# izhengfan/se2lam

Hardware: AMD Instinct MI355X
Metric: BA GN-iters/s (200 KF, 20k pts) (higher is better)
Workload: dtype f64; 1 GPU; globalBA-window 200 KF / 20000 landmarks / 119817 EdgeSE2XYZ + 199 PreEdgeSE2, LM optimize(10) (config 4 formulation, SURVEY D3); parallelism=single GPU

## Files before the change

include/se2gpu.h:

```cpp
#ifndef SE2GPU_H
#define SE2GPU_H

#include <stddef.h>
#include <stdint.h>

#ifdef __cplusplus
extern "C" {
#endif

#define SE2GPU_OK 0
#define SE2GPU_ERR_INVALID (-1)
#define SE2GPU_ERR_NO_DEVICE (-2)
#define SE2GPU_ERR_HIP (-3)
#define SE2GPU_ERR_CAPACITY (-4)
#define SE2GPU_ERR_STATE (-5)

const char* se2gpu_last_error(void);
int se2gpu_device_count(void);
const char* se2gpu_version(void);

typedef struct se2gpu_orb se2gpu_orb;

typedef struct se2gpu_orb_params {
    int32_t nfeatures;
// ... 88 lines not shown
int se2gpu_ba_clear(se2gpu_ba* h);
int se2gpu_ba_set_stream(se2gpu_ba* h, void* hip_stream);
int se2gpu_ba_add_cam(se2gpu_ba* h, double f, double cx, double cy);
int se2gpu_ba_set_Tbc(se2gpu_ba* h, const double R[9], const double t[3]);
int se2gpu_ba_add_vertex_se2(se2gpu_ba* h, int id, double x, double y, double theta, int fixed);
int se2gpu_ba_add_vertex_xyz(se2gpu_ba* h, int id, const double xyz[3], int marginal, int fixed);
int se2gpu_ba_add_edge_se2xyz(se2gpu_ba* h, int id_kf, int id_mp, const double uv[2], const double info[4],
                              double huber_delta);
int se2gpu_ba_add_edge_se2(se2gpu_ba* h, int id0, int id1, const double meas[3], const double info[9]);

int se2gpu_ba_load(se2gpu_ba* h, int P, int L, int E, int O,
                   const double* poses, const uint8_t* fixed, const double* lms,
                   const int32_t* e_kf, const int32_t* e_lm, const double* e_uv, const double* e_info,
                   const int32_t* o_i, const int32_t* o_j, const double* o_meas, const double* o_info,
                   double huber_delta);

int se2gpu_ba_add_vertex_se3(se2gpu_ba* h, int id, const double pose12[12], int fixed);
int se2gpu_ba_add_vertex_iso3(se2gpu_ba* h, int id, const double Twc12[12], int fixed);
int se2gpu_plane_motion_prior_iso3(const double* Twc12, const double* Tbc12, double xrot_info, double yrot_info,
                                   double z_info, double* meas12, double* info36);
int se2gpu_ba_add_prior_se3(se2gpu_ba* h, int id, const double meas12[12], const double info36[36]);
int se2gpu_ba_add_edge_se3(se2gpu_ba* h, int id0, int id1, const double meas12[12], const double info36[36]);
int se2gpu_ba_add_edge_xyz2uv(se2gpu_ba* h, int id_mp, int id_kf, const double uv[2], double inv_sigma2, double huber_delta);
int se2gpu_ba_get_se3(se2gpu_ba* h, int id, double pose12[12]);
int se2gpu_ba_edge_chi2(se2gpu_ba* h, double* chi2, int cap);

int se2gpu_sparsify_se3xyz(int npairs, const double* kf12, const int32_t* mp_ptr, const double* mp_xyz,
                           const int32_t* m_ptr, const int32_t* m_kf, const int32_t* m_mp, const double* m_info,
                           double* z_out12, double* info_out36);

typedef struct se2gpu_local_graph {
    int32_t n_local_kf, n_ref_kf, n_mp, n_obs;
    const int32_t* kf_id;
    const float* kf_Twb;
    const float* kf_Rcw;
    const int32_t* odo_to;
    const double* odo_meas;
    const double* odo_cov;
    const float* mp_pos;
    const int32_t* obs_mp;
    const int32_t* obs_kf;
    const float* obs_uv;
    const float* obs_lc;
    const float* obs_sigma2;
    float fx, cx, cy;
    double Rbc[9], tbc[3];
    float huber_delta;
    float xrot_info, z_info;
} se2gpu_local_graph;
int se2gpu_ba_load_local_graph(se2gpu_ba* h, const se2gpu_local_graph* graph);

typedef struct se2gpu_map_view {
    int32_t n_kf, n_mp;
    const int32_t* kf_id;
    const int32_t* covis_ptr; const int32_t* covis_idx;
    const int32_t* kf_mp_ptr; const int32_t* kf_mp_idx;
    const int32_t* mp_id;
    const int32_t* mp_kf_ptr; const int32_t* mp_kf_idx;
} se2gpu_map_view;
int se2gpu_map_update_local_graph(const se2gpu_map_view* map, int current_kf, int search_level, int32_t* local_kfs,
                                  int* n_local, int32_t* ref_kfs, int* n_ref, int32_t* local_mps, int* n_mps);

int se2gpu_ba_initialize(se2gpu_ba* h);
int se2gpu_ba_set_edge_level(se2gpu_ba* h, int edge, int level);
int se2gpu_ba_reset_estimates(se2gpu_ba* h);
int se2gpu_ba_reset_estimates_batch(se2gpu_ba** handles, int count);

#define SE2GPU_BA_LM 0
#define SE2GPU_BA_GN 1
int se2gpu_ba_optimize(se2gpu_ba* h, int iters, int mode, const volatile uint8_t* stop_flag, int verbose,
                       se2gpu_ba_stats* stats);
int se2gpu_ba_optimize_batch(se2gpu_ba** handles, int count, int iters, int mode, const volatile uint8_t* stop_flag,
                             se2gpu_ba_stats* stats);
int se2gpu_ba_last_batch_path(void);
int se2gpu_ba_get_se2(se2gpu_ba* h, int id, double xyt[3]);
int se2gpu_ba_get_xyz(se2gpu_ba* h, int id, double xyz[3]);
int se2gpu_ba_get_all(se2gpu_ba* h, double* poses , double* lms );
double se2gpu_ba_chi2(se2gpu_ba* h);

int se2gpu_ba_debug_reduced_system(se2gpu_ba* h, double lambda, double* S, double* bs);
int se2gpu_ba_debug_solve(se2gpu_ba* h, double lambda, double* x, int* factor_ok);
int se2gpu_ba_debug_solver_path(const se2gpu_ba* h);
int se2gpu_ba_debug_linearize_counts(const se2gpu_ba* h, int* runs, int* skips, long long* twin_bytes);
int se2gpu_ba_debug_pool_sizes(int out2[2]);
int se2gpu_ba_debug_chol_verify(se2gpu_ba* h, unsigned long long* counts2, unsigned long long* records, int cap);
int se2gpu_ba_debug_solve_plan(int P, int D, const uint8_t* pattern, int allow_nd, int* nsys, int* nbc, int* depth, int* ntask,
                               int* ndep, int32_t* pose_off, int32_t* tasks4, int task_cap, int32_t* deps, int dep_cap);
int se2gpu_ba_debug_solve_plan_tile(int P, int D, const uint8_t* pattern, int allow_nd, int tile, int* nsys, int* nbc, int* depth, int* ntask,
                                    int* ndep, int32_t* pose_off, int32_t* tasks4, int task_cap, int32_t* deps, int dep_cap);

int se2gpu_triangulate(int n, const se2gpu_keypoint* kps_ref, const se2gpu_keypoint* kps_cur, int n_cur,
                       int32_t* match_idx, const uint8_t* has_observation, const float* P_ref, const float* P_cur,
                       const float* Ocam, float lower_depth, float upper_depth, int min_degree, float* pos_out,
                       uint8_t* good_parallax, int* n_good, int* n_tracked_old);

typedef struct se2gpu_track se2gpu_track;
int se2gpu_track_create(se2gpu_track** out);
void se2gpu_track_destroy(se2gpu_track* h);
int se2gpu_track_fundamental_mask(se2gpu_track* h, const float* pt1, const float* pt2, int n, uint8_t* mask,
                                  int* n_inliers);
int se2gpu_track_remove_outliers(se2gpu_track* h, const se2gpu_keypoint* kps1, int n1, const se2gpu_keypoint* kps2,
                                 int n2, int32_t* matches, int* n_inliers);
int se2gpu_track_last_ransac(const se2gpu_track* h, int info[4]);
int se2gpu_track_triangulate(se2gpu_track* h, int n, const se2gpu_keypoint* kps_ref, const se2gpu_keypoint* kps_cur,
                             int n_cur, int32_t* match_idx, const uint8_t* has_observation, const float* P_ref,
                             const float* P_cur, const float* Ocam, float lower_depth, float upper_depth,
                             int min_degree, float* pos_out, uint8_t* good_parallax, int* n_good, int* n_tracked_old);

int se2gpu_plane_motion_prior(const double* Tcw12, const double* Tbc12, double xrot_info, double yrot_info, double z_info,
                              double* meas12, double* info36);
int se2gpu_track_pose_ba(se2gpu_track* h, const double* Tcw12, const double* prior_meas12, const double* prior_info36, int n,
                         const double* xyz, const double* uv, const double* inv_sigma2, double f, double cx, double cy,
                         double huber_delta, int iters, double* Tcw_out12, se2gpu_ba_stats* stats);

int se2gpu_ba_edge_information(int E, const float* lc, const float* lw, const int32_t* e_kf, const float* sigma2, int P,
                               const float* Rcw, const float* twb_xy, float fx, float xrot_info, float z_info,
                               double* info_out);

typedef int (*se2gpu_allreduce_fn)(void* dev_ptr, size_t count_doubles, void* hip_stream, void* user);
size_t se2gpu_ba_reduce_buffer_doubles(se2gpu_ba* h, int P);
size_t se2gpu_ba_exchange_doubles(int P);
size_t se2gpu_ba_exchange_doubles_h(const se2gpu_ba* h);
int se2gpu_ba_exchange_row(int row, size_t* offset, int* length);
int se2gpu_ba_set_allreduce(se2gpu_ba* h, se2gpu_allreduce_fn fn, void* user, void* buffer);
int se2gpu_ba_set_shard(se2gpu_ba* h, int rank, int world);

typedef struct se2gpu_comm se2gpu_comm;
int se2gpu_comm_unique_id(uint8_t id_out[128]);
int se2gpu_comm_create(const uint8_t id[128], int rank, int world, se2gpu_comm** out);
int se2gpu_comm_count(se2gpu_comm* c, int* nranks);
void se2gpu_comm_destroy(se2gpu_comm* c);
int se2gpu_comm_allreduce_sum_f64(se2gpu_comm* c, void* dev_ptr, size_t count, void* hip_stream);
int se2gpu_ba_set_comm(se2gpu_ba* h, se2gpu_comm* c);

int se2gpu_ba_shard_landmarks(int L, int E, const int32_t* e_kf, const int32_t* e_lm, int world, int32_t* owner);

typedef struct se2gpu_timer se2gpu_timer;
int se2gpu_timer_create(se2gpu_timer** out);
void se2gpu_timer_destroy(se2gpu_timer* t);
int se2gpu_timer_start(se2gpu_timer* t, void* hip_stream);
int se2gpu_timer_stop(se2gpu_timer* t, void* hip_stream);
int se2gpu_timer_elapsed_ms(se2gpu_timer* t, float* ms);
void* se2gpu_orb_stream(se2gpu_orb* h);
void* se2gpu_matcher_stream(se2gpu_matcher* h);
void* se2gpu_ba_stream(se2gpu_ba* h);
int se2gpu_ba_profile(se2gpu_ba* h, int enable);
int se2gpu_ba_profile_get(se2gpu_ba* h, int idx, const char** name, double* ms, int64_t* launches);
int se2gpu_orb_score_kernel(se2gpu_orb* h, int info[2]);
int se2gpu_orb_profile(se2gpu_orb* h, int enable);
int se2gpu_orb_profile_get(se2gpu_orb* h, int idx, const char** name, double* ms, int64_t* launches);

int se2gpu_malloc(void** dev_ptr, size_t bytes);
int se2gpu_free(void* dev_ptr);
int se2gpu_memcpy_h2d(void* dst, const void* src, size_t bytes);
int se2gpu_memcpy_d2h(void* dst, const void* src, size_t bytes);
int se2gpu_device_synchronize(void);
int se2gpu_set_device(int ordinal);
int se2gpu_host_alloc(void** host_ptr, size_t bytes);
int se2gpu_host_free(void* host_ptr);
int se2gpu_memcpy_h2d_async(void* dst, const void* src, size_t bytes, void* hip_stream);
int se2gpu_memcpy_d2h_async(void* dst, const void* src, size_t bytes, void* hip_stream);
int se2gpu_stream_create(void** hip_stream_out);
int se2gpu_stream_destroy(void* hip_stream);
int se2gpu_stream_synchronize(void* hip_stream);
int se2gpu_timer_stream_wait(se2gpu_timer* t, void* hip_stream);

// ... 5 lines not shown
```

se2lam_amd/capi.py:

```python
from __future__ import annotations

import ctypes as C
import os

import numpy as np

HERE = os.path.dirname(os.path.abspath(__file__))
LIB_PATH = os.path.join(HERE, "lib", "libse2gpu.so")

OK = 0
ERR_INVALID, ERR_NO_DEVICE, ERR_HIP, ERR_CAPACITY, ERR_STATE = -1, -2, -3, -4, -5


class Se2GpuError(RuntimeError):
    def __init__(self, code, msg):
        super().__init__(f"se2gpu error {code}: {msg}")
        self.code = code


class Keypoint(C.Structure):
    _fields_ = [("x", C.c_float), ("y", C.c_float), ("size", C.c_float), ("angle", C.c_float),
                ("response", C.c_float), ("octave", C.c_int32), ("class_id", C.c_int32)]


# ... 35 lines not shown
                ("lambda_final", C.c_double), ("chi2_hist", C.c_double * 64), ("lambda_hist", C.c_double * 64),
                ("trials_hist", C.c_int32 * 64)]


ALLREDUCE_FN = C.CFUNCTYPE(C.c_int, C.c_void_p, C.c_size_t, C.c_void_p, C.c_void_p)

_VP, _I, _D, _F, _SZ = C.c_void_p, C.c_int, C.c_double, C.c_float, C.c_size_t
_PD, _PI32, _PU8, _PF = C.POINTER(C.c_double), C.POINTER(C.c_int32), C.POINTER(C.c_uint8), C.POINTER(C.c_float)
_PKP = C.POINTER(Keypoint)
SYMBOLS = {
    "se2gpu_last_error": (C.c_char_p, []),
    "se2gpu_device_count": (_I, []),
    "se2gpu_version": (C.c_char_p, []),
    "se2gpu_orb_create": (_I, [C.POINTER(OrbParams), C.POINTER(_VP)]),
    "se2gpu_orb_destroy": (None, [_VP]),
    "se2gpu_orb_levels": (_I, [_VP]),
    "se2gpu_orb_scale_factor": (_F, [_VP]),
    "se2gpu_orb_extract": (_I, [_VP, _VP, _I, _I, _SZ, _VP, _VP, _VP, _I, C.POINTER(_I)]),
    "se2gpu_orb_extract_batch_device": (_I, [_VP, _VP, _I, _I, _I, _VP, _VP, _VP, _I]),
    "se2gpu_orb_sync": (_I, [_VP]),
    "se2gpu_orb_set_stream": (_I, [_VP, _VP]),
    "se2gpu_orb_debug_level": (_I, [_VP, _I, _I, _I, _VP, _SZ, C.POINTER(_I), C.POINTER(_I)]),
    "se2gpu_orb_debug_score": (_I, [_VP, _I, _I, _VP, _SZ, C.POINTER(_I), C.POINTER(_I)]),
    "se2gpu_orb_debug_nth_element": (_I, [_VP, _I, _I, _I]),
    "se2gpu_orb_stream": (_VP, [_VP]),
    "se2gpu_orb_score_kernel": (_I, [_VP, _VP]),
    "se2gpu_orb_profile": (_I, [_VP, _I]),
    "se2gpu_orb_profile_get": (_I, [_VP, _I, C.POINTER(C.c_char_p), _PD, C.POINTER(C.c_int64)]),
    "se2gpu_hamming": (_I, [_VP, _VP]),
    "se2gpu_three_maxima": (_I, [_VP, _I, _VP, _VP, _VP]),
    "se2gpu_matcher_create": (_I, [_I, _I, C.POINTER(_VP)]),
    "se2gpu_matcher_destroy": (None, [_VP]),
    "se2gpu_matcher_set_stream": (_I, [_VP, _VP]),
    "se2gpu_matcher_sync": (_I, [_VP]),
    "se2gpu_matcher_spill_calls": (_I, [_VP, _VP]),
    "se2gpu_matcher_stream": (_VP, [_VP]),
    "se2gpu_match_window": (_I, [_VP, C.POINTER(FrameBounds), _VP, _VP, _I, _VP, _VP, _I, _VP, _I, _I, _I, _I, _F,
                                 _VP, C.POINTER(_I)]),
    "se2gpu_match_window_batch_device": (_I, [_VP, C.POINTER(FrameBounds), _VP, _VP, _VP, _I, _VP, _VP, _I, _I, _I,
                                              _I, _I, _F, _VP, _VP]),
    "se2gpu_search_by_bow": (_I, [_VP, _VP, _VP, _I, _VP, _VP, _VP, _I, _VP, _VP, _VP, _I, _VP, _VP, _VP, _I, _VP, _I, _F, _I,
                                  _VP, C.POINTER(_I)]),
    "se2gpu_match_projection": (_I, [_VP, C.POINTER(FrameBounds), _VP, _VP, _VP, _VP, _I, _VP, _F, _F, _F, _F,
                                     _VP, _VP, _VP, _I, _I, _I, _F, _VP, C.POINTER(_I)]),
    "se2gpu_ba_create": (_I, [C.POINTER(_VP)]),
    "se2gpu_ba_reserve": (_I, [_I, _I, _I]),
    "se2gpu_ba_destroy": (None, [_VP]),
    "se2gpu_ba_clear": (_I, [_VP]),
    "se2gpu_ba_set_stream": (_I, [_VP, _VP]),
    "se2gpu_ba_stream": (_VP, [_VP]),
    "se2gpu_ba_add_cam": (_I, [_VP, _D, _D, _D]),
    "se2gpu_ba_set_Tbc": (_I, [_VP, _PD, _PD]),
    "se2gpu_ba_add_vertex_se2": (_I, [_VP, _I, _D, _D, _D, _I]),
    "se2gpu_ba_add_vertex_xyz": (_I, [_VP, _I, _PD, _I, _I]),
    "se2gpu_ba_add_edge_se2xyz": (_I, [_VP, _I, _I, _PD, _PD, _D]),
    "se2gpu_ba_add_edge_se2": (_I, [_VP, _I, _I, _PD, _PD]),
    "se2gpu_ba_load": (_I, [_VP, _I, _I, _I, _I, _PD, _PU8, _PD, _PI32, _PI32, _PD, _PD, _PI32, _PI32, _PD, _PD, _D]),
    "se2gpu_ba_load_local_graph": (_I, [_VP, C.POINTER(LocalGraph)]),
    "se2gpu_ba_add_vertex_se3": (_I, [_VP, _I, _PD, _I]),
    "se2gpu_ba_add_vertex_iso3": (_I, [_VP, _I, _PD, _I]),
    "se2gpu_plane_motion_prior_iso3": (_I, [_VP, _VP, _D, _D, _D, _VP, _VP]),
    "se2gpu_ba_add_prior_se3": (_I, [_VP, _I, _PD, _PD]),
    "se2gpu_ba_add_edge_se3": (_I, [_VP, _I, _I, _PD, _PD]),
    "se2gpu_ba_add_edge_xyz2uv": (_I, [_VP, _I, _I, _PD, _D, _D]),
    "se2gpu_ba_get_se3": (_I, [_VP, _I, _PD]),
    "se2gpu_ba_edge_chi2": (_I, [_VP, _PD, _I]),
    "se2gpu_map_update_local_graph": (_I, [C.POINTER(MapView), _I, _I, _VP, C.POINTER(_I), _VP, C.POINTER(_I), _VP, C.POINTER(_I)]),
    "se2gpu_sparsify_se3xyz": (_I, [_I, _VP, _VP, _VP, _VP, _VP, _VP, _VP, _VP, _VP]),
    "se2gpu_ba_initialize": (_I, [_VP]),
    "se2gpu_ba_set_edge_level": (_I, [_VP, _I, _I]),
    "se2gpu_ba_reset_estimates": (_I, [_VP]),
    "se2gpu_ba_reset_estimates_batch": (_I, [_VP, _I]),
    "se2gpu_ba_optimize": (_I, [_VP, _I, _I, _PU8, _I, C.POINTER(BaStats)]),
    "se2gpu_ba_optimize_batch": (_I, [C.POINTER(_VP), _I, _I, _I, _PU8, C.POINTER(BaStats)]),
    "se2gpu_ba_last_batch_path": (_I, []),
    "se2gpu_ba_get_se2": (_I, [_VP, _I, _PD]),
    "se2gpu_ba_get_xyz": (_I, [_VP, _I, _PD]),
    "se2gpu_ba_get_all": (_I, [_VP, _PD, _PD]),
    "se2gpu_ba_chi2": (_D, [_VP]),
    "se2gpu_ba_debug_reduced_system": (_I, [_VP, _D, _PD, _PD]),
    "se2gpu_ba_debug_solve": (_I, [_VP, _D, _PD, C.POINTER(C.c_int)]),
    "se2gpu_ba_debug_solver_path": (_I, [_VP]),
    "se2gpu_ba_debug_linearize_counts": (_I, [_VP, C.POINTER(C.c_int), C.POINTER(C.c_int), C.POINTER(C.c_longlong)]),
    "se2gpu_ba_debug_chol_verify": (_I, [_VP, _VP, _VP, _I]),
    "se2gpu_ba_debug_pool_sizes": (_I, [_VP]),
    "se2gpu_ba_debug_solve_plan": (_I, [_I, _I, _VP, _I, _VP, _VP, _VP, _VP, _VP, _VP, _VP, _I, _VP, _I]),
    "se2gpu_ba_debug_solve_plan_tile": (_I, [_I, _I, _VP, _I, _I, _VP, _VP, _VP, _VP, _VP, _VP, _VP, _I, _VP, _I]),
    "se2gpu_triangulate": (_I, [_I, _VP, _VP, _I, _VP, _VP, _VP, _VP, _VP, C.c_float, C.c_float, _I, _VP, _VP,
                           C.POINTER(C.c_int), C.POINTER(C.c_int)]),
    "se2gpu_track_create": (_I, [C.POINTER(_VP)]),
    "se2gpu_track_destroy": (None, [_VP]),
    "se2gpu_track_fundamental_mask": (_I, [_VP, _VP, _VP, _I, _VP, C.POINTER(C.c_int)]),
    "se2gpu_track_remove_outliers": (_I, [_VP, _VP, _I, _VP, _I, _VP, C.POINTER(C.c_int)]),
    "se2gpu_track_last_ransac": (_I, [_VP, _VP]),
    "se2gpu_plane_motion_prior": (_I, [_VP, _VP, _D, _D, _D, _VP, _VP]),
    "se2gpu_track_pose_ba": (_I, [_VP, _VP, _VP, _VP, _I, _VP, _VP, _VP, _D, _D, _D, _D, _I, _VP, C.POINTER(BaStats)]),
    "se2gpu_track_triangulate": (_I, [_VP, _I, _VP, _VP, _I, _VP, _VP, _VP, _VP, _VP, C.c_float, C.c_float, _I, _VP, _VP,
                                 C.POINTER(C.c_int), C.POINTER(C.c_int)]),
    "se2gpu_ba_reduce_buffer_doubles": (_SZ, [_VP, _I]),
    "se2gpu_ba_exchange_doubles": (_SZ, [_I]),
    "se2gpu_ba_exchange_doubles_h": (_SZ, [_VP]),
    "se2gpu_ba_exchange_row": (_I, [_I, C.POINTER(C.c_size_t), C.POINTER(C.c_int)]),
    "se2gpu_ba_set_allreduce": (_I, [_VP, ALLREDUCE_FN, _VP, _VP]),
    "se2gpu_ba_set_shard": (_I, [_VP, _I, _I]),
    "se2gpu_comm_unique_id": (_I, [_VP]),
    "se2gpu_comm_create": (_I, [_VP, _I, _I, C.POINTER(_VP)]),
    "se2gpu_comm_destroy": (None, [_VP]),
    "se2gpu_comm_count": (_I, [_VP, C.POINTER(_I)]),
    "se2gpu_comm_allreduce_sum_f64": (_I, [_VP, _VP, _SZ, _VP]),
    "se2gpu_ba_set_comm": (_I, [_VP, _VP]),
    "se2gpu_ba_shard_landmarks": (_I, [_I, _I, _PI32, _PI32, _I, _PI32]),
    "se2gpu_ba_edge_information": (_I, [_I, _VP, _VP, _VP, _VP, _I, _VP, _VP, _F, _F, _F, _VP]),
    "se2gpu_ba_profile": (_I, [_VP, _I]),
    "se2gpu_ba_profile_get": (_I, [_VP, _I, C.POINTER(C.c_char_p), _PD, C.POINTER(C.c_int64)]),
    "se2gpu_timer_create": (_I, [C.POINTER(_VP)]),
    "se2gpu_timer_destroy": (None, [_VP]),
    "se2gpu_timer_start": (_I, [_VP, _VP]),
    "se2gpu_timer_stop": (_I, [_VP, _VP]),
    "se2gpu_timer_elapsed_ms": (_I, [_VP, C.POINTER(C.c_float)]),
    "se2gpu_malloc": (_I, [C.POINTER(_VP), _SZ]),
    "se2gpu_free": (_I, [_VP]),
    "se2gpu_memcpy_h2d": (_I, [_VP, _VP, _SZ]),
    "se2gpu_memcpy_d2h": (_I, [_VP, _VP, _SZ]),
    "se2gpu_host_alloc": (_I, [C.POINTER(_VP), _SZ]),
    "se2gpu_host_free": (_I, [_VP]),
    "se2gpu_memcpy_h2d_async": (_I, [_VP, _VP, _SZ, _VP]),
    "se2gpu_memcpy_d2h_async": (_I, [_VP, _VP, _SZ, _VP]),
    "se2gpu_stream_create": (_I, [C.POINTER(_VP)]),
    "se2gpu_stream_destroy": (_I, [_VP]),
    "se2gpu_stream_synchronize": (_I, [_VP]),
    "se2gpu_timer_stream_wait": (_I, [_VP, _VP]),
    "se2gpu_device_synchronize": (_I, []),
    "se2gpu_set_device": (_I, [_I]),
}

_lib = None


def lib() -> C.CDLL:
    global _lib
    if _lib is None:
        if not os.path.exists(LIB_PATH):
            raise ImportError(
                f"{LIB_PATH} is missing - run `python -m se2lam_amd.build` (or __graft_entry__.build()). "
                "se2lam_amd has no CPU / eager fallback.")
        l = C.CDLL(LIB_PATH)
        for name, (res, args) in SYMBOLS.items():
            fn = getattr(l, name)
            fn.restype = res
            fn.argtypes = args
        _lib = l
    return _lib


def check(rc: int):
    if rc != OK:
        raise Se2GpuError(rc, lib().se2gpu_last_error().decode(errors="replace"))


def device_count() -> int:
    return int(lib().se2gpu_device_count())


def vp(a: np.ndarray) -> C.c_void_p:
    return C.c_void_p(a.ctypes.data)

# ... 100 lines not shown
```

se2lam_amd/csrc/ba.hip:

```cpp
#include <algorithm>
#include <atomic>
#include <chrono>
#include <cmath>
#include <cstdlib>
#include <functional>
#include <limits>
#include <mutex>
#include <thread>
#include <tuple>
#include <memory>
#include <unordered_map>

#include "common.h"
#include "se3_math.h"
#include "ba_device.h"
#include "ba3_device.h"
#include "ba_window.h"

using namespace se2gpu;
using namespace se2gpu::badev;

namespace {


// ... 839 lines not shown
        __syncthreads();
    } else {
        t0 = *reinterpret_cast<const double2*>(ownp);
        t1 = *reinterpret_cast<const double2*>(ownp + 2);
        const double* dp = A + (size_t)r * ld + cc;
        d0 = *reinterpret_cast<const double2*>(dp);
        d1 = *reinterpret_cast<const double2*>(dp + 2);
        if (!elim) return;
    }
    Ti[r][cc] = t0.x; Ti[r][cc + 1] = t0.y; Ti[r][cc + 2] = t1.x; Ti[r][cc + 3] = t1.y;
    Tj[r][cc] = d0.x; Tj[r][cc + 1] = d0.y; Tj[r][cc + 2] = d1.x; Tj[r][cc + 3] = d1.y;
    __syncthreads();
    if (tid >= 64) return;
    const int lane = tid;
    const int c0 = kNB * k;
    const int ncol = min(kNB, n - c0);
    const int rr = lane & 31;
    double m[kNB];
    {
        const double* lp = (lane < kNB) ? &Tj[rr][0] : &Ti[rr][0];
        const bool ident = isDiag && lane >= kNB;
#pragma unroll
        for (int c = 0; c < kNB; c += 2) {
            const double2 v = *reinterpret_cast<const double2*>(lp + c);
            m[c] = ident ? (c == rr ? 1.0 : 0.0) : v.x;
            m[c + 1] = ident ? (c + 1 == rr ? 1.0 : 0.0) : v.y;
        }
#pragma unroll
        for (int c = 0; c < kNB; ++c)
            if (c >= ncol) m[c] = (lane < kNB && c == rr) ? 1e300 : 0.0;
    }
    double inv = fast_rcp(bcast_lane(m[0], 0));
#pragma unroll
    for (int jj = 0; jj < kNB; ++jj) {
        const double mr = m[jj] * inv;
        if (jj + 1 < kNB) {
            m[jj + 1] = fma(-mr, bcast_lane(m[jj], jj + 1), m[jj + 1]);
            inv = fast_rcp(bcast_lane(m[jj + 1], jj + 1));
        }
        if (jj + 2 < kNB) {
            double* col = (jj & 1) ? colB : colA;
            col[lane] = m[jj];
#pragma unroll
            for (int c = jj + 2; c < kNB; ++c) m[c] = fma(-mr, col[c], m[c]);
        }
    }
    bool bad = false;
    double out[kNB];
#pragma unroll
    for (int c = 0; c < kNB; ++c) {
        const double d = bcast_lane(m[c], c);
        const bool pos = (d > 0.0) & (d < __builtin_inf());
        bad |= (c < ncol) & !pos;
        out[c] = m[c] * fast_rsqrt(((c < ncol) & pos) ? d : 1.0);
    }
    double* rowp;
    if (lane < kNB) rowp = A + (size_t)(c0 + rr) * ld + c0;
    else if (isDiag) rowp = R + (size_t)(c0 + rr) * ld + c0;
    else rowp = own + (size_t)(kNB * i + rr) * ld + c0;
    if (ncol == kNB) {
        if (lane >= kNB) {
            double2* wp2 = reinterpret_cast<double2*>(rowp);
#pragma unroll
            for (int c = 0; c < kNB; c += 2) wp2[c / 2] = make_double2(out[c], out[c + 1]);
        }
    } else {
#pragma unroll
        for (int c = 0; c < kNB; ++c)
            if (c < ncol && (lane >= kNB || (isDiag && rr >= ncol))) rowp[c] = out[c];
    }
    if (bad && isDiag && lane == 0) fail[0] = 1.0;
}

typedef double d2_t __attribute__((ext_vector_type(2)));
typedef double d4_t __attribute__((ext_vector_type(4)));
__device__ inline d2_t load_agent(const double* p) {
    d2_t v;
    asm volatile("global_load_dwordx4 %0, %1, off sc1" : "=v"(v) : "v"(p) : "memory");
    return v;
}
__device__ inline void store_agent(double* p, d2_t v) {
    asm volatile("global_store_dwordx4 %0, %1, off sc1\n\ts_nop 1" : : "v"(p), "v"(v) : "memory");
}
#define SE2_WAIT_VM6(a, b, c, d, e, f) \
    asm volatile("s_waitcnt vmcnt(0)" : "+v"(a), "+v"(b), "+v"(c), "+v"(d), "+v"(e), "+v"(f) : : "memory")

__device__ inline unsigned poll_agent(const unsigned* p) {
    unsigned v;
    asm volatile("global_load_dword %0, %1, off sc1" : "=v"(v) : "v"(p) : "memory");
    return v;
}
__device__ inline bool spin_until(const unsigned* f, unsigned epoch, bool lazy = false) {
    if (__hip_atomic_load(f, __ATOMIC_RELAXED, __HIP_MEMORY_SCOPE_AGENT) == epoch) return true;
    const long long t0 = wall_clock64();
    while (__hip_atomic_load(f, __ATOMIC_RELAXED, __HIP_MEMORY_SCOPE_AGENT) != epoch) {
        if (lazy) __builtin_amdgcn_s_sleep(48);
        else __builtin_amdgcn_s_sleep(2);
        if (wall_clock64() - t0 > 200000000ll) return false;
    }
    return true;
}

constexpr int kVfyRecords = 64, kVfyChk = 8 + 8 * kVfyRecords;
__device__ inline unsigned long long wave_xor64(unsigned long long v) {
#pragma unroll
    for (int m = 1; m < 64; m <<= 1) v ^= (unsigned long long)__shfl_xor((long long)v, m);
    return v;
}
__device__ inline unsigned long long bits4(d2_t a, d2_t b) {
    return (unsigned long long)__double_as_longlong(a.x) ^ (unsigned long long)__double_as_longlong(a.y) ^
           (unsigned long long)__double_as_longlong(b.x) ^ (unsigned long long)__double_as_longlong(b.y);
}
template <bool VERIFY>
__device__ __forceinline__ void d_chol_tiles(const unsigned bx_dispatch, const double* __restrict__ A, double* __restrict__ PUB,
                                                     double* __restrict__ YU, int ld, int n,
                                                     int nbc, const int4* __restrict__ tasks, const int* __restrict__ deps,
                                                     const int* __restrict__ col_src,
                                                     unsigned* __restrict__ flagA, unsigned* __restrict__ flagR,
                                                     const unsigned* __restrict__ epoch_ptr, double* __restrict__ fail,
                                                     long long* __restrict__ dbg, const BaCtl* __restrict__ ctl,
                                                     double* __restrict__ xout, unsigned long long* __restrict__ vfy,
                                                     unsigned long long* __restrict__ head, int ntask) {
    if (ctl && ctl->done) return;
    __shared__ unsigned task_s;
    if (head) {
        if (threadIdx.x == 0) {
            const unsigned c = __hip_atomic_fetch_add(reinterpret_cast<unsigned*>(head), 1u, __ATOMIC_RELAXED, __HIP_MEMORY_SCOPE_AGENT);
            if (c == (unsigned)ntask - 1u) __hip_atomic_store(reinterpret_cast<unsigned*>(head), 0u, __ATOMIC_RELAXED, __HIP_MEMORY_SCOPE_AGENT);
            task_s = c;
        }
        __syncthreads();
    }
    const unsigned bx = head ? task_s : bx_dispatch;
    const unsigned epoch = *epoch_ptr;
    const int nt = ld / kNB;
    constexpr int kTile = kNB * (kNB + 2);
    __shared__ __attribute__((aligned(16))) double LD[3 * kTile + kNB * kNB + 8 * kNB];
    double (*Tb)[kNB + 2] = reinterpret_cast<double (*)[kNB + 2]>(LD);
    double (*Tc)[kNB + 2] = reinterpret_cast<double (*)[kNB + 2]>(LD + kTile);
    double (*Ta)[kNB + 2] = reinterpret_cast<double (*)[kNB + 2]>(LD + 2 * kTile);
    double (*COLV)[kNB] = reinterpret_cast<double (*)[kNB]>(LD + 3 * kTile);
    double* const DUMMY = LD + 3 * kTile + kNB * kNB;
    double (*MRC)[64] = reinterpret_cast<double (*)[64]>(LD + kTile);
    static_assert(16 * 64 <= kTile && 32 * 64 <= 2 * kTile, "rows 0..15 of MRC lie inside Tc, all of it inside Tc | Ta");
    __shared__ int ok_s, ready_s, loaded_s, slab_s[kSlabs];
    __shared__ int deps_s[64];
    const int tid = threadIdx.x;
    if (tid == 0) { ready_s = 0; loaded_s = 0; ok_s = 1; }
    if (tid < kSlabs) slab_s[tid] = 0;
    long long* stamp = dbg ? dbg + (size_t)bx * 16 : nullptr;
    if (stamp && tid == 0) stamp[0] = wall_clock64();
    const int4 tk = tasks[bx];
    if (tid < tk.w - tk.z && tid < 64) deps_s[tid] = deps[tk.z + tid];
    __syncthreads();
    if ((tk.x >> 16) == 2) {
        const int r = tk.x & 0xffff;
        const int it = n / kNB;
        const int row = tid / 8, c4 = (tid % 8) * 4;
        double acc = 0.0;
        for (int dq = tk.z; dq < tk.w; ++dq) {
            const int j = deps_s[dq - tk.z];
            if (tid == 0) {
                const bool lazy = dq + 1 < tk.w;
                bool ok = true;
                for (int sl = 0; sl < kSlabs; ++sl) {
                    ok = ok && spin_until(flagR + ((size_t)r * nbc + j) * kSlabs + sl, epoch, lazy);
// ... 227 lines not shown
    if (stamp && tid == 224) stamp[6] = clock64() - clk0;
    if (lane >= kNB) {
        double* pb = PUB + pub_tile(isR || isDiag ? 1 : 0, i, j, nt, nbc) + w * kSlabDoubles + rr * 2;
#pragma unroll
        for (int q = 0; q < 8; q += 2) {
            store_agent(pb + q * kNB, d2_t{m[q], m[q + 1]});
            store_agent(pb + kSlabDoubles / 2 + q * kNB, d2_t{mrs[q], mrs[q + 1]});
        }
    }
    if constexpr (VERIFY) {
        unsigned long long xm = 0, xr = 0;
        if (lane >= kNB) {
#pragma unroll
            for (int q = 0; q < 8; ++q) {
                xm ^= (unsigned long long)__double_as_longlong(m[q]);
                xr ^= (unsigned long long)__double_as_longlong(mrs[q]);
            }
        }
        xm = wave_xor64(xm);
        xr = wave_xor64(xr);
        if (lane == 0) {
            const size_t tx = ((size_t)((isR || isDiag ? 1 : 0) * nt + i) * nbc + j) * kSlabs + w;
            __hip_atomic_store(vfy + kVfyChk + 2 * tx, xm, __ATOMIC_RELAXED, __HIP_MEMORY_SCOPE_AGENT);
            __hip_atomic_store(vfy + kVfyChk + 2 * tx + 1, xr, __ATOMIC_RELAXED, __HIP_MEMORY_SCOPE_AGENT);
        }
    }
    if (!isR && i == n / kNB && lane == (isDiag ? 0 : kNB) + n % kNB) {
#pragma unroll
        for (int q = 0; q < 8; q += 2) store_agent(YU + c0 + cb + q, d2_t{m[q], m[q + 1]});
    }
    if (bad && isDiag && lane == 0) fail[0] = 1.0;
    asm volatile("s_waitcnt vmcnt(0)" ::: "memory");
    if (lane == 0)
        __hip_atomic_store((isR || isDiag ? flagR : flagA) + ((size_t)i * nbc + j) * kSlabs + w, epoch, __ATOMIC_RELAXED, __HIP_MEMORY_SCOPE_AGENT);
    if (stamp && lane == 0) stamp[12 + w] = wall_clock64();
    if (stamp && tid == 192) stamp[5] = wall_clock64();
}
template <bool VERIFY>
__global__ __launch_bounds__(256) void k_chol_tiles(const double* __restrict__ A, double* __restrict__ PUB,
                                                     double* __restrict__ YU, int ld, int n,
                                                     int nbc, const int4* __restrict__ tasks, const int* __restrict__ deps,
                                                     const int* __restrict__ col_src,
                                                     unsigned* __restrict__ flagA, unsigned* __restrict__ flagR,
                                                     const unsigned* __restrict__ epoch_ptr, double* __restrict__ fail,
                                                     long long* __restrict__ dbg, const BaCtl* __restrict__ ctl,
                                                     double* __restrict__ xout, unsigned long long* __restrict__ vfy,
                                                     unsigned long long* __restrict__ head, int ntask) {
    d_chol_tiles<VERIFY>(blockIdx.x, A, PUB, YU, ld, n, nbc, tasks, deps, col_src, flagA, flagR, epoch_ptr, fail, dbg, ctl, xout, vfy, head, ntask);
}

__global__ __launch_bounds__(256) void k_chol_apply(const double* __restrict__ A, const double* __restrict__ R, int ld,
                                                     int n, double* __restrict__ x, const BaCtl* __restrict__ ctl,
                                                     const int* __restrict__ col_src) {
    if (ctl && ctl->done) return;
    const int r = blockIdx.x * 4 + threadIdx.x / 64;
    const int lane = threadIdx.x & 63;
    if (r >= n) return;
    const double* y = A + (size_t)n * ld;
    double acc = 0.0;
    for (int c = r + lane; c < n; c += 64) acc += R[(size_t)r * ld + c] * y[c];
    acc = wave_sum(acc);
    const int dst = col_src ? col_src[r] : r;
    if (lane == 0 && dst >= 0) x[dst] = acc;
}

struct FinArgs {
    int enabled, nblk, P, O, root, step, decide, notify;
    const uint8_t* fixed;
    const double* xp;
    const double* bp;
    const double* poses;
    double* poses_trial;
    const int* o_i;
    const int* o_j;
    const double* o_meas;
    const double* o_info;
    double* out;
    volatile double* mail;
    double seq;
    BaCtl* ctl;
    const volatile int* stop;
    unsigned* counter;
    int spec;
};
__device__ void finish_trial(const FinArgs& fin, const double* part, double lambda, double* fsp);

struct SpecArgs {
    RecSet set[2];
    double *Hpp_e, *bp_e;
};

template <bool LIN>
__device__ __forceinline__ void d_update(const unsigned bx, CamDev cam, int L, double lambda, const int* __restrict__ lm_ptr,
                                                    const int* __restrict__ e_kf, const double* __restrict__ e_uv,
                                                    const double* __restrict__ e_info,
                                                    const double* __restrict__ poses,
                                                    const uint8_t* __restrict__ fixed, const double* __restrict__ lms,
                                                    const double* __restrict__ xp, const double* __restrict__ zeta,
                                                    const double* __restrict__ W, const double* __restrict__ bl,
                                                    double* __restrict__ lms_trial, double* __restrict__ part,
                                                    const BaCtl* __restrict__ ctl, const double* __restrict__ poses_b,
                                                    FinArgs fin, const double* __restrict__ Ainv, SpecArgs sp) {
    __shared__ double lds[LIN ? (kBlock / 64) * kWaveLds : 3 * 1024];
    static_assert((kBlock / 64) * kWaveLds >= 3 * 1024, "the finisher's pose stage");
    if (fin.enabled && (int)bx == fin.nblk) {
        finish_trial(fin, part, lambda, lds);
        return;
    }
    const int gid = bx * kBlock + threadIdx.x;
    const int l = gid / kGroup, sub = gid % kGroup;
    int beg = 0, end = 0;
    if (l < L) {
        beg = lm_ptr[l];
        end = lm_ptr[l + 1];
    }
    if (ctl) {
        if (ctl->done) return;
        if (ctl->sel) {
            const double* t = lms; lms = lms_trial; lms_trial = const_cast<double*>(t);
            poses = poses_b;
        }
        lambda = ctl->lambda;
    }
    const bool step = xp != nullptr;
    bool spec = false;
    double lambda_spec = 0;
    RecSet wr{};
    if (LIN && ctl && step) {
        spec = ctl->it + 1 < ctl->iters;
        lambda_spec = lm_lambda_spec(lambda, ctl->mode);
        const int rs = ctl->rec_sel;
        const RecSet rd = sp.set[rs];
        wr = sp.set[rs ^ 1];
        W = rd.W; zeta = rd.zeta; bl = rd.bl; Ainv = rd.Ainv;
    }
    double* keep = lds;
    double hll[6] = {0, 0, 0, 0, 0, 0}, bsum[3] = {0, 0, 0};
    __shared__ double sm[2][kBlock / 64];
    double chi = 0, scale = 0;
    double x[3] = {0, 0, 0};
    constexpr int KS = 2;
    int ekf[KS];
    bool ev[KS];
    double ey[KS][9], ep[KS][3], epose[KS][3], euv[KS][2], ew[KS][3];
    bool efix[KS];
#pragma unroll
    for (int k = 0; k < KS; ++k) {
        const int e = beg + sub + k * kGroup;
        ev[k] = e < end;
        const int ec = ev[k] ? e : max(end - 1, 0);
        const bool has = l < L && end > beg;
        ekf[k] = has ? e_kf[ec] : 0;
#pragma unroll
        for (int i = 0; i < 9; ++i) ey[k][i] = (has && step) ? W[(size_t)ec * 9 + i] : 0.0;
        euv[k][0] = has ? e_uv[2 * (size_t)ec] : 0.0;
        euv[k][1] = has ? e_uv[2 * (size_t)ec + 1] : 0.0;
#pragma unroll
        for (int i = 0; i < 3; ++i) ew[k][i] = has ? e_info[3 * (size_t)ec + i] : 0.0;
    }
#pragma unroll
    for (int k = 0; k < KS; ++k) {
        const int kf = ekf[k];
        epose[k][0] = poses[3 * kf]; epose[k][1] = poses[3 * kf + 1]; epose[k][2] = poses[3 * kf + 2];
        efix[k] = fixed[kf] != 0;
#pragma unroll
        for (int i = 0; i < 3; ++i) ep[k][i] = step ? xp[3 * kf + i] : 0.0;
    }
    double lw0[3] = {0, 0, 0}, zz[3] = {0, 0, 0}, blv[3] = {0, 0, 0}, av[6] = {0, 0, 0, 0, 0, 0};
    if (l < L) {
#pragma unroll
        for (int c = 0; c < 3; ++c) {
            lw0[c] = lms[(size_t)l * 3 + c];
            if (step) { zz[c] = zeta[(size_t)l * 3 + c]; blv[c] = bl[(size_t)l * 3 + c]; }
        }
        if (step) {
#pragma unroll
            for (int c = 0; c < 6; ++c) av[c] = Ainv[(size_t)l * 6 + c];
        }
    }
    if (l < L && step) {
#pragma unroll
        for (int k = 0; k < KS; ++k)
            if (ev[k]) {
#pragma unroll
                for (int c = 0; c < 3; ++c) x[c] -= ey[k][c] * ep[k][0] + ey[k][3 + c] * ep[k][1] + ey[k][6 + c] * ep[k][2];
            }
        for (int e = beg + sub + KS * kGroup; e < end; e += kGroup) {
            const int kf = e_kf[e];
            const double* y = W + (size_t)e * 9;
            const double p0 = xp[3 * kf], p1 = xp[3 * kf + 1], p2 = xp[3 * kf + 2];
#pragma unroll
            for (int c = 0; c < 3; ++c) x[c] -= y[c] * p0 + y[3 + c] * p1 + y[6 + c] * p2;
        }
    }
#pragma unroll
    for (int c = 0; c < 3; ++c) x[c] = group_sum(x[c]);
    if (l < L && step) {
        const double t0 = zz[0] + x[0], t1 = zz[1] + x[1], t2 = zz[2] + x[2];
        x[0] = av[0] * t0 + av[1] * t1 + av[3] * t2;
        x[1] = av[2] * t1 + av[4] * t2;
        x[2] = av[5] * t2;
    }
    if (l < L) {
        double lw[3];
#pragma unroll
        for (int c = 0; c < 3; ++c) lw[c] = lw0[c] + x[c];
        if (sub == 0 && step) {
#pragma unroll
            for (int c = 0; c < 3; ++c) {
                lms_trial[(size_t)l * 3 + c] = lw[c];
                scale += x[c] * (lambda * x[c] + blv[c]);
            }
        }
        auto edge_chi = [&](int e, double px, double py, double pth, bool fx, const double* dp, double u, double v, double w0,
                            double w1, double w2) {
            if (step && !fx) {
                px += dp[0];
                py += dp[1];
                pth = normalize_theta(pth + dp[2]);
            }
            if (LIN && spec) {
                double hpl[9], hpp[6], bpe[3], r0;
                lin_edge(cam, px, py, pth, lw[0], lw[1], lw[2], u, v, w0, w1, w2, !fx, hll, bsum, hpl, hpp, bpe, r0);
                chi += r0;
                lin_park<true>(e == beg + sub, e, hpl, hpp, bpe, keep, wr.W, sp.Hpp_e, sp.bp_e);
                return;
            }
            double e0, e1;
            se2xyz<false>(cam, px, py, pth, lw[0], lw[1], lw[2], u, v, e0, e1, nullptr, nullptr);
            double r0, r1;
            huber(e0 * (w0 * e0 + w1 * e1) + e1 * (w1 * e0 + w2 * e1), cam.huber, r0, r1);
            chi += r0;
        };
#pragma unroll
        for (int k = 0; k < KS; ++k)
            if (ev[k]) edge_chi(beg + sub + k * kGroup, epose[k][0], epose[k][1], epose[k][2], efix[k], ep[k], euv[k][0], euv[k][1], ew[k][0], ew[k][1], ew[k][2]);
        for (int e = beg + sub + KS * kGroup; e < end; e += kGroup) {
            const int kf = e_kf[e];
            double dp[3] = {0, 0, 0};
            if (step) { dp[0] = xp[3 * kf]; dp[1] = xp[3 * kf + 1]; dp[2] = xp[3 * kf + 2]; }
            edge_chi(e, poses[3 * kf], poses[3 * kf + 1], poses[3 * kf + 2], fixed[kf] != 0, dp, e_uv[2 * e], e_uv[2 * e + 1],
                     e_info[3 * e], e_info[3 * e + 1], e_info[3 * e + 2]);
        }
    }
    chi = wave_sum(chi);
    scale = wave_sum(scale);
    const int w = threadIdx.x / 64;
    if ((threadIdx.x & 63) == 0) { sm[0][w] = chi; sm[1][w] = scale; }
    __syncthreads();
    if (threadIdx.x == 0) {
        double c = 0, s = 0;
        for (int i = 0; i < kBlock / 64; ++i) { c += sm[0][i]; s += sm[1][i]; }
        if (fin.enabled) {
            store_agent(part + 2 * bx, d2_t{c, s});
            asm volatile("s_waitcnt vmcnt(0)" ::: "memory");
            __hip_atomic_fetch_add(fin.counter, 1u, __ATOMIC_RELAXED, __HIP_MEMORY_SCOPE_AGENT);
        } else {
            part[2 * bx] = c;
            part[2 * bx + 1] = s;
        }
    }
    if (LIN && spec)
        lin_landmark<true>(l, sub, beg, end, L, hll, bsum, lambda_spec, keep, wr.W, sp.Hpp_e, sp.bp_e, wr.Hll, wr.bl, wr.Ainv,
                           wr.zeta, wr.Dg);
}
template <bool LIN>
__global__ __launch_bounds__(kBlock) void k_update(CamDev cam, int L, double lambda, const int* __restrict__ lm_ptr,
                                                    const int* __restrict__ e_kf, const double* __restrict__ e_uv,
                                                    const double* __restrict__ e_info,
                                                    const double* __restrict__ poses,
                                                    const uint8_t* __restrict__ fixed, const double* __restrict__ lms,
                                                    const double* __restrict__ xp, const double* __restrict__ zeta,
                                                    const double* __restrict__ W, const double* __restrict__ bl,
                                                    double* __restrict__ lms_trial, double* __restrict__ part,
                                                    const BaCtl* __restrict__ ctl, const double* __restrict__ poses_b,
                                                    FinArgs fin, const double* __restrict__ Ainv, SpecArgs sp) {
    d_update<LIN>(blockIdx.x, cam, L, lambda, lm_ptr, e_kf, e_uv, e_info, poses, fixed, lms, xp, zeta, W, bl, lms_trial, part, ctl, poses_b, fin, Ainv, sp);
}


__global__ void k_ctl_clear_error(BaCtl* __restrict__ ctl) {
    ctl->error = 0;
    ctl->done = 0;
}

__device__ inline void post_ctl(const BaCtl* c, volatile double* mail, double seq, int tid, int nthr) {
    constexpr int kWords = (int)(sizeof(BaCtl) / 8);
    const double* src = reinterpret_cast<const double*>(c);
    for (int i = tid; i < kWords; i += nthr) mail[8 + i] = src[i];
}

__device__ inline void end_slot(BaCtl* ctl, volatile double* mail, bool post, int tid, int nthr, bool step) {
    if (!step) return;
    if (tid == 0) ctl->seq += 1.0;
    __syncthreads();
    if (post && mail) {
        __threadfence();
        post_ctl(ctl, mail, 0.0, tid, nthr);
        __threadfence_system();
        __syncthreads();
        if (tid == 0) mail[kMailSeq] = ctl->seq;
    }
}

__device__ void finish_trial(const FinArgs& fin, const double* part, double lambda, double* fsp) {
    __shared__ double fsm[2][kBlock / 64];
    __shared__ int fpost;
    BaCtl* ctl = fin.ctl;
    const volatile double* cmail = fin.mail;
    volatile double* mail = fin.mail;
    (void)cmail;
    const double* poses = fin.poses;
    double* poses_trial = fin.poses_trial;
    const bool step = fin.step != 0;
    int stopped = 0;
    double failflag = 0;
    if (ctl) {
        if (ctl->done) {
            end_slot(ctl, mail, fin.notify != 0, threadIdx.x, blockDim.x, fin.step != 0);
            return;
        }
        if (ctl->sel) { const double* t = poses; poses = poses_trial; poses_trial = const_cast<double*>(t); }
        lambda = ctl->lambda;
    }
    if (threadIdx.x == 0) {
        stopped = (fin.stop && *fin.stop) ? 1 : 0;
        failflag = step ? fin.out[2] : 0.0;
    }
    double chi = 0, scale = 0;
    for (int p = threadIdx.x; p < fin.P; p += blockDim.x) {
        double x = poses[3 * p], y = poses[3 * p + 1], th = poses[3 * p + 2];
        if (step && !fin.fixed[p]) {
            const double d0 = fin.xp[3 * p], d1 = fin.xp[3 * p + 1], d2 = fin.xp[3 * p + 2];
            x += d0; y += d1; th = normalize_theta(th + d2);
            const double* bp = fin.bp;
            if (fin.root) scale += d0 * (lambda * d0 + bp[3 * p]) + d1 * (lambda * d1 + bp[3 * p + 1]) + d2 * (lambda * d2 + bp[3 * p + 2]);
            else scale += d0 * bp[3 * p] + d1 * bp[3 * p + 1] + d2 * bp[3 * p + 2];
        }
        if (step) { poses_trial[3 * p] = x; poses_trial[3 * p + 1] = y; poses_trial[3 * p + 2] = th; }
        if (p < 1024) { fsp[3 * p] = x; fsp[3 * p + 1] = y; fsp[3 * p + 2] = th; }
    }
    __syncthreads();
    for (int k = threadIdx.x; k < fin.O; k += blockDim.x) {
        const int i = fin.o_i[k], j = fin.o_j[k];
        double pi[3], pj[3];
        for (int c = 0; c < 3; ++c) {
            pi[c] = (i < 1024) ? fsp[3 * i + c] : (step ? poses_trial[3 * i + c] : poses[3 * i + c]);
            pj[c] = (j < 1024) ? fsp[3 * j + c] : (step ? poses_trial[3 * j + c] : poses[3 * j + c]);
        }
        double e[3], A[9], B[9];
        pre_se2(pi, pj, fin.o_meas + 3 * k, e, A, B);
        const double* W = fin.o_info + 9 * k;
        for (int r = 0; r < 3; ++r) chi += e[r] * (W[r * 3] * e[0] + W[r * 3 + 1] * e[1] + W[r * 3 + 2] * e[2]);
    }
    if (threadIdx.x == 0) {
        const long long t0 = wall_clock64();
        while (__hip_atomic_load(fin.counter, __ATOMIC_RELAXED, __HIP_MEMORY_SCOPE_AGENT) != (unsigned)fin.nblk) {
            __builtin_amdgcn_s_sleep(1);
            if (wall_clock64() - t0 > 200000000ll) break;
        }
        __hip_atomic_store(fin.counter, 0u, __ATOMIC_RELAXED, __HIP_MEMORY_SCOPE_AGENT);
    }
    __syncthreads();
    for (int i0 = threadIdx.x; i0 < fin.nblk; i0 += 4 * blockDim.x) {
        d2_t v[4];
#pragma unroll
        for (int u = 0; u < 4; ++u) v[u] = load_agent(part + 2 * min(i0 + u * (int)blockDim.x, fin.nblk - 1));
        asm volatile("s_waitcnt vmcnt(0)" : "+v"(v[0]), "+v"(v[1]), "+v"(v[2]), "+v"(v[3]) : : "memory");
#pragma unroll
        for (int u = 0; u < 4; ++u)
            if (i0 + u * (int)blockDim.x < fin.nblk) { chi += v[u].x; scale += v[u].y; }
    }
    chi = wave_sum(chi);
    scale = wave_sum(scale);
    if ((threadIdx.x & 63) == 0) {
        fsm[0][threadIdx.x >> 6] = chi;
        fsm[1][threadIdx.x >> 6] = scale;
    }
    __syncthreads();
    if (threadIdx.x == 0) {
        for (int w = 1; w < (int)(blockDim.x >> 6); ++w) {
            fsm[0][0] += fsm[0][w];
            fsm[1][0] += fsm[1][w];
        }
        double* out = fin.out;
        out[0] = fsm[0][0]; out[1] = fsm[1][0]; out[3] = 0;
        if (!step) out[2] = 0;
        fpost = 0;
        if (ctl && fin.decide) {
            if (!step) {
                ctl->current_chi = ctl->chi2_init = ctl->chi2_final = fsm[0][0];
                if (stopped) { ctl->stopped = 1; ctl->done = 1; }
                if (ctl->iters <= 0) ctl->done = 1;
            } else {
                const double sc[3] = {fsm[0][0], fsm[1][0], failflag};
                const int sel0 = ctl->sel;
                const bool speculated = fin.spec && ctl->it + 1 < ctl->iters;
                const double lambda_spec = lm_lambda_spec(ctl->lambda, ctl->mode);
                lm_advance(ctl, sc, stopped != 0);
                if (!ctl->error) lm_records_advance(ctl, speculated, sel0, lambda_spec);
            }
            fpost = (ctl->done || fin.notify) && mail;
        } else if (mail && !ctl) {
            mail[0] = fsm[0][0];
            mail[1] = fsm[1][0];
            mail[2] = step ? failflag : 0.0;
            __threadfence_system();
            mail[3] = fin.seq;
        }
    }
    if (ctl && fin.decide) {
        __syncthreads();
        end_slot(ctl, mail, fpost != 0, threadIdx.x, blockDim.x, step);
    }
}

__global__ void k_finalize(int nparts, const double* __restrict__ part, int P, double lambda,
                           const double* __restrict__ poses, const uint8_t* __restrict__ fixed,
                           const double* __restrict__ xp, const double* __restrict__ bp, double* __restrict__ poses_trial,
                           int O, const int* __restrict__ o_i, const int* __restrict__ o_j,
                           const double* __restrict__ o_meas, const double* __restrict__ o_info, int root,
                           double* __restrict__ out, volatile double* __restrict__ mail, double seq,
                           BaCtl* __restrict__ ctl, int step_arg, int decide, int notify,
                           const volatile int* __restrict__ stop) {
    __shared__ double sm[2][16];
    __shared__ double sp[3 * 1024];
    __shared__ int post_s;
    bool step = xp != nullptr;
    if (ctl) {
        step = step_arg != 0;
        if (ctl->done) {
            if (decide) end_slot(ctl, mail, notify != 0, threadIdx.x, blockDim.x, step);
            return;
        }
        if (ctl->sel) { const double* t = poses; poses = poses_trial; poses_trial = const_cast<double*>(t); }
        lambda = ctl->lambda;
    }
    double chi = 0, scale = 0;
    for (int i = threadIdx.x; i < nparts; i += blockDim.x) {
        chi += part[2 * i];
        scale += part[2 * i + 1];
    }
    for (int p = threadIdx.x; p < P; p += blockDim.x) {
        double x = poses[3 * p], y = poses[3 * p + 1], th = poses[3 * p + 2];
        if (step && !fixed[p]) {
            const double d0 = xp[3 * p], d1 = xp[3 * p + 1], d2 = xp[3 * p + 2];
            x += d0; y += d1; th = normalize_theta(th + d2);
            if (root) scale += d0 * (lambda * d0 + bp[3 * p]) + d1 * (lambda * d1 + bp[3 * p + 1]) + d2 * (lambda * d2 + bp[3 * p + 2]);
            else scale += d0 * bp[3 * p] + d1 * bp[3 * p + 1] + d2 * bp[3 * p + 2];
        }
        if (step) { poses_trial[3 * p] = x; poses_trial[3 * p + 1] = y; poses_trial[3 * p + 2] = th; }
        if (p < 1024) { sp[3 * p] = x; sp[3 * p + 1] = y; sp[3 * p + 2] = th; }
    }
    __syncthreads();
    for (int k = threadIdx.x; k < O; k += blockDim.x) {
        const int i = o_i[k], j = o_j[k];
        double pi[3], pj[3];
        for (int c = 0; c < 3; ++c) {
            pi[c] = (i < 1024) ? sp[3 * i + c] : (step ? poses_trial[3 * i + c] : poses[3 * i + c]);
            pj[c] = (j < 1024) ? sp[3 * j + c] : (step ? poses_trial[3 * j + c] : poses[3 * j + c]);
        }
        double e[3], A[9], B[9];
        pre_se2(pi, pj, o_meas + 3 * k, e, A, B);
        const double* W = o_info + 9 * k;
        for (int r = 0; r < 3; ++r) chi += e[r] * (W[r * 3] * e[0] + W[r * 3 + 1] * e[1] + W[r * 3 + 2] * e[2]);
    }
    chi = wave_sum(chi);
    scale = wave_sum(scale);
    if ((threadIdx.x & 63) == 0) {
        sm[0][threadIdx.x >> 6] = chi;
        sm[1][threadIdx.x >> 6] = scale;
    }
    __syncthreads();
    if (threadIdx.x == 0) {
        for (int w = 1; w < (int)(blockDim.x >> 6); ++w) {
            sm[0][0] += sm[0][w];
            sm[1][0] += sm[1][w];
        }
        out[0] = sm[0][0]; out[1] = sm[1][0]; out[3] = 0;
        if (!step) out[2] = 0;
        post_s = 0;
        if (ctl && decide) {
            if (!step) {
// ... 868 lines not shown
    int find(int id) const {
        if ((unsigned)id < dense.size()) return dense[(unsigned)id];
        if ((unsigned)id < kDenseIds) return -1;
        const auto it = sparse.find(id);
        return it == sparse.end() ? -1 : it->second;
    }
    void set(int id, int slot) {
        if ((unsigned)id < kDenseIds) {
            if ((unsigned)id >= dense.size()) dense.resize(std::max<size_t>((size_t)id + 1, 2 * dense.size()), -1);
            dense[(unsigned)id] = slot;
        } else {
            sparse[id] = slot;
        }
    }
    void clear() { dense.clear(); sparse.clear(); }
    void reserve(size_t n) { dense.reserve(n); }
};

constexpr int kMailDoubles = 256, kMailStop = 250;
static_assert(8 + sizeof(BaCtl) / 8 <= kMailStop, "controller block does not fit the mailbox");

inline std::atomic<unsigned long>& streams_destroyed() { static std::atomic<unsigned long> n{0}; return n; }

struct se2gpu_ba {
    hipStream_t own_stream = nullptr, stream = nullptr;
    LaunchProfile prof;
    CamDev cam{};
    bool have_cam = false, have_tbc = false;
    double Rbc[9] = {1, 0, 0, 0, 1, 0, 0, 0, 1}, tbc[3] = {0, 0, 0};
    IdTable pose_of_id, lm_of_id;
    std::vector<int> pose_ids, lm_ids;
    std::vector<double> h_poses, h_lms;
    std::vector<uint8_t> h_fixed;
    std::vector<int> he_kf, he_lm;
    std::vector<double> he_uv, he_info;
    double huber_delta = 0;
    bool huber_mixed = false;
    int model = 0, D = 3, ps = 3;
    Cam3 cam3{};
    std::vector<uint8_t> h_prior_has;
    std::vector<double> h_prior_meas, h_prior_info;
    struct Odo3 { int i, j; double meas[12], info[36]; int level = 0; };
    std::vector<Odo3> odo3;
    DevBuf<uint8_t> prior_has;
    DevBuf<double> prior_meas, prior_info, pb, edge_chi2;
    std::vector<int> edge_perm;
    int pg_edges = 0;
    std::vector<int> pg_perm;
    DevBuf<int> slot_a, slot_ptr, pe_i, pe_j;
    DevBuf<double> pe_meas, pe_info, ph;
    int bulk_E = 0;
    const int32_t *bulk_kf = nullptr, *bulk_lm = nullptr;
    const double *bulk_uv = nullptr, *bulk_info = nullptr;
    bool lg_active = false;
    std::vector<float> lg_lc, lg_lw, lg_sigma2, lg_Rcw, lg_twb;
    float lg_fx = 0, lg_srot = 0, lg_sz = 0;
    DevBuf<float> d_lg_lc, d_lg_lw, d_lg_sigma2, d_lg_Rcw, d_lg_twb;
    std::vector<EdgeOdo> odo;
    bool initialized = false;
    unsigned long init_serial = 0;
    hipEvent_t join_event = nullptr;
    hipStream_t join_stream = nullptr;
    bool own_pending = false;
    int P = 0, L = 0, E = 0, O = 0, nblk = 0, nparts = 0;
    int ld = 0;
    bool host_solve = false;
    DevBuf<double> poses0, lms0, poses_a, poses_b, lms_a, lms_b;
    double *poses = nullptr, *poses_t = nullptr, *lms = nullptr, *lms_t = nullptr;
    DevBuf<uint8_t> fixed;
    DevBuf<int> lm_ptr, e_kf, e_lm, pose_ptr, pose_edges, podo_ptr, podo_item, o_i, o_j;
    DevBuf<int> blk_a, blk_b, blk_ptr, pair_i, pair_j, blk_odo;
    DevBuf<int4> grp;
    int nwg_off = 0, grp_cap_wg = 0;
    DevBuf<uint8_t> garena;
    DevBuf<int> plan_np, plan_base, plan_key0, plan_key1, plan_idx, plan_hist, plan_offs, plan_out, plan_tsum, plan_toff;
    DevBuf<int2> plan_st0, plan_st1;
    bool odo_fallback = false;
    bool odo_self_loop = false;
    DevBuf<double> e_uv, e_info, o_meas, o_info;
    DevBuf<double> Hpl, Hpp_e, bp_e, Hll, bl, Dinv, z, Y, Dg, Hpp, bp, Oii, Ojj, Oij, obi, obj;
    DevBuf<double> red_own, xp, part, scal, diag3, Rinv;
    DevBuf<double> rec_twin;
    bool run_spec = false;
    DevBuf<double> red_packed;
    DevBuf<int4> chol_tasks;
    DevBuf<int> chol_deps;
    DevBuf<int> pose_off;
    DevBuf<int> col_src;
    std::vector<int> h_pose_off;
    DevBuf<uint8_t> plan_nz;
    DevBuf<double> plan_nzd;
    PinBuf<uint8_t> h_plan_nz;
    DevBuf<uint8_t> solver_arena;
    int nsys = 0;
    int solve_depth = 0;
    DevBuf<unsigned> chol_flags;
    DevBuf<unsigned long long> chol_head;
    DevBuf<unsigned long long> chol_vfy;
    DevBuf<int> plan_place;
    DevBuf<unsigned> fin_counter;
    DevBuf<unsigned long long> l0_acc;
    int chol_ntask = 0;
    struct GraphSlot { int iters = -1, mode = -1; hipGraphExec_t exec = nullptr; unsigned long stamp = 0; };
    static constexpr int kGraphSlots = 3;
    GraphSlot graphs[kGraphSlots];
    unsigned long graph_clock = 0;
    void drop_graphs() {
        for (auto& g : graphs) {
            if (g.exec) (void)hipGraphExecDestroy(g.exec);
            g = GraphSlot{};
        }
    }
    double dev_seq = 0;
    DevBuf<long long> chol_trace;
    bool chol_steps = false;
    bool chol_faulted = false;
    bool chol_fallback = false;
    double* red = nullptr;
    PinBuf<double> h_red, h_x, h_scal;
    double* h_mail = nullptr;
    double* d_mail = nullptr;
    volatile int* h_stop = nullptr;
    int* d_stop = nullptr;
    uint64_t mail_seq = 0;
    DevBuf<BaCtl> ctl;
    int run_mode = SE2GPU_BA_LM, run_iters = 0, run_enqueued = 0;
    bool run_sync = false, run_active = false;
    double run_seq = 0;
    se2gpu_allreduce_fn allreduce = nullptr;
    void* ar_user = nullptr;
    se2gpu_comm* comm = nullptr;
    void* ar_buffer = nullptr;
    int root = 1, rank = 0, world = 1;
    int device = 0;
    PinBuf<uint8_t> h_stage;
    PinBuf<uint8_t> h_stage_solver;
    PinBuf<double> est;
    bool est_valid = false;

    hipEvent_t ev_copy0 = nullptr, ev_copy1 = nullptr, ev_pat = nullptr;

    ~se2gpu_ba() {
        if (ev_copy0) (void)hipEventDestroy(ev_copy0);
        if (ev_copy1) (void)hipEventDestroy(ev_copy1);
        if (ev_pat) (void)hipEventDestroy(ev_pat);
        drop_graphs();
        if (own_stream) {
            (void)hipStreamDestroy(own_stream);
            streams_destroyed().fetch_add(1, std::memory_order_relaxed);
        }
        if (h_mail) (void)hipHostFree(h_mail);
    }
};

namespace {

__device__ __host__ inline int blk_index_of(int P, int a, int b) { return a * P - a * (a - 1) / 2 + (b - a); }

__global__ __launch_bounds__(1024) void k_scan_i32(const int* __restrict__ in, int* __restrict__ out, int n) {
    __shared__ int wtot[16];
    const int t = threadIdx.x, lane = t & 63, wave = t >> 6;
    const int per = (n + 1023) / 1024;
    const int b = min(t * per, n), e = min(b + per, n);
    constexpr int kKeep = 32;
    int v[kKeep];
    int s = 0;
    if (per <= kKeep) {
#pragma unroll
        for (int u = 0; u < kKeep; ++u) v[u] = (u < per && b + u < e) ? in[b + u] : 0;
#pragma unroll
        for (int u = 0; u < kKeep; ++u) s += v[u];
    } else {
        for (int i = b; i < e; ++i) s += in[i];
    }
    int inc = s;
#pragma unroll
    for (int off = 1; off < 64; off <<= 1) {
        const int o = __shfl_up(inc, off);
        if (lane >= off) inc += o;
    }
    if (lane == 63) wtot[wave] = inc;
    __syncthreads();
    int base = 0;
    for (int w = 0; w < wave; ++w) base += wtot[w];
    int run = base + inc - s;
    if (per <= kKeep) {
// ... 1160 lines not shown
        SE2_HIP(hipMemsetAsync(h->chol_flags.p, 0, 2 * kSlabs * (size_t)nt2 * nbc2 * sizeof(unsigned), st));
        SE2_CHECK(h->chol_head.reserve(1));
        SE2_HIP(hipMemsetAsync(h->chol_head.p, 0, sizeof(unsigned long long), st));
        static const bool verify = env_flag("SE2GPU_BA_CHOL_VERIFY", false);
        if (verify) {
            const size_t words = kVfyChk + 2 * 2 * kSlabs * (size_t)nt2 * nbc2;
            SE2_CHECK(h->chol_vfy.reserve(words));
            SE2_HIP(hipMemsetAsync(h->chol_vfy.p, 0, words * sizeof(unsigned long long), st));
        } else {
            h->chol_vfy.release();
        }
        h->chol_steps = env_is("SE2GPU_BA_CHOL", "steps") || nt2 > 64 || h->chol_fallback;
        if (env_flag("SE2GPU_BA_CHOL_TRACE", false)) {
            SE2_CHECK(h->chol_trace.reserve(16 * (size_t)h->chol_ntask));
            SE2_HIP(hipMemsetAsync(h->chol_trace.p, 0, 16 * (size_t)h->chol_ntask * sizeof(long long), st));
        }
        lap("solve plan");
    }
    SE2_HIP(hipStreamSynchronize(st));
    if (device_plan) {
        int nwg = 0;
        std::memcpy(&nwg, h->h_scal.p, sizeof(int));
        SE2_REQUIRE(nwg <= h->grp_cap_wg, SE2GPU_ERR_CAPACITY, "device plan: %d workgroups exceed the bound %d", nwg, h->grp_cap_wg);
        h->nwg_off = std::max(nwg, 1);
    }
    lap("synchronise");
    h->bulk_E = 0;
    h->bulk_kf = h->bulk_lm = nullptr;
    h->bulk_uv = h->bulk_info = nullptr;
    h->initialized = true;
    h->est_valid = false;
    static std::atomic<unsigned long> serial{0};
    h->init_serial = ++serial;
    drain.armed = false;
    return SE2GPU_OK;
}


int ba_join(se2gpu_ba* h, hipStream_t st, hipEvent_t* ev) {
    if (h->join_event) {
        if (h->join_stream != st) SE2_HIP(hipStreamWaitEvent(st, h->join_event, 0));
        h->join_event = nullptr;
        h->join_stream = nullptr;
    }
    if (h->own_pending && h->stream != st) {
        if (!*ev) SE2_HIP(hipEventCreateWithFlags(ev, hipEventDisableTiming));
        SE2_HIP(hipEventRecord(*ev, h->stream));
        SE2_HIP(hipStreamWaitEvent(st, *ev, 0));
        h->own_pending = false;
    }
    return SE2GPU_OK;
}
inline int ba_join(se2gpu_ba* h) { return ba_join(h, h->stream, nullptr); }
struct ResetItem {
    double* dst_p; const double* src_p; unsigned np;
    double* dst_l; const double* src_l; unsigned nl;
};
__global__ __launch_bounds__(256) void k_reset_one(double* __restrict__ poses, const double* __restrict__ poses0, size_t np,
                                                    double* __restrict__ lms, const double* __restrict__ lms0, size_t nl) {
    const size_t i = (size_t)blockIdx.x * 256 + threadIdx.x;
    if (i < np) poses[i] = poses0[i];
    if (i < nl) lms[i] = lms0[i];
}
__global__ __launch_bounds__(256) void k_reset_batch(const ResetItem* __restrict__ items) {
    const ResetItem it = items[blockIdx.y];
    const unsigned stride = gridDim.x * 256, t0 = blockIdx.x * 256 + threadIdx.x;
    for (unsigned i = t0; i < it.np; i += stride) it.dst_p[i] = it.src_p[i];
    for (unsigned i = t0; i < it.nl; i += stride) it.dst_l[i] = it.src_l[i];
}

struct Bufs {
    const BaCtl* c;
    double *pa, *pb, *la, *lb;
};
inline Bufs bufs(se2gpu_ba* h, bool ctl) {
    if (ctl) return Bufs{h->ctl.p, h->poses_a.p, h->poses_b.p, h->lms_a.p, h->lms_b.p};
    return Bufs{nullptr, h->poses, h->poses_t, h->lms, h->lms_t};
}

bool ba_env_speculate() {
    static const bool on = env_flag("SE2GPU_BA_SPECULATE", true);
    return on;
}
RecSet rec_own(const se2gpu_ba* h) { return RecSet{h->Hpl.p, h->Dg.p, h->Hll.p, h->bl.p, h->Dinv.p, h->z.p}; }
RecSet rec_twin(const se2gpu_ba* h) {
    if (!h->rec_twin.p || h->model) return RecSet{};
    const size_t E = (size_t)h->E, L = (size_t)h->L;
    double* p = h->rec_twin.p;
    RecSet r;
    r.W = p; p += 9 * E + 1;
    r.Dg = p; p += 12 * E + 1;
    r.Hll = p; p += 6 * L + 1;
    r.bl = p; p += 3 * L + 1;
    r.Ainv = p; p += 6 * L + 1;
    r.zeta = p;
    return r;
}
int ba_reserve_twin(se2gpu_ba* h) { return h->rec_twin.reserve(21 * (size_t)h->E + 18 * (size_t)h->L + 6); }


int ba_linearize(se2gpu_ba* h, double fuse_lambda, bool ctl = false) {
    hipStream_t st = h->stream;
    const Bufs B = bufs(h, ctl);
    if (h->model == 2) {
        SE2_LAUNCH(h->prof, st, "k4_terms", k4_terms, grid1((size_t)h->P + h->O, 64), dim3(64), 0, h->P, h->O, B.pa, h->fixed.p,
                   h->prior_has.p, h->prior_meas.p, h->prior_info.p, h->ph.p, h->pb.p, h->slot_a.p, h->slot_ptr.p, h->pe_i.p,
                   h->pe_j.p, h->pe_meas.p, h->pe_info.p, h->Oii.p, h->Ojj.p, h->Oij.p, h->obi.p, h->obj.p, B.c, B.pb);
        SE2_HIP(hipGetLastError());
        return SE2GPU_OK;
    }
    if (h->model) {
        if (fuse_lambda >= 0.0)
            SE2_LAUNCH(h->prof, st, "k3_linearize", (k3_linearize<true>), grid1((size_t)h->L * kGroup, kBlock), dim3(kBlock), 0,
                       h->cam3, h->L, h->lm_ptr.p, h->e_kf.p, h->e_uv.p, h->e_info.p, B.pa, h->fixed.p, B.la, h->Hpl.p,
                       h->Hpp_e.p, h->bp_e.p, h->Hll.p, h->bl.p, fuse_lambda, h->Dinv.p, h->z.p, h->Y.p, h->Dg.p, B.c, B.pb, B.lb);
        else
            SE2_LAUNCH(h->prof, st, "k3_linearize", (k3_linearize<false>), grid1((size_t)h->L * kGroup, kBlock), dim3(kBlock), 0,
                       h->cam3, h->L, h->lm_ptr.p, h->e_kf.p, h->e_uv.p, h->e_info.p, B.pa, h->fixed.p, B.la, h->Hpl.p,
                       h->Hpp_e.p, h->bp_e.p, h->Hll.p, h->bl.p, 0.0, h->Dinv.p, h->z.p, h->Y.p, h->Dg.p, B.c, B.pb, B.lb);
        SE2_LAUNCH(h->prof, st, "k3_terms", k3_terms, grid1((size_t)h->P + h->O, 64), dim3(64), 0, h->P, h->O, B.pa, h->fixed.p,
                   h->prior_has.p, h->prior_meas.p, h->prior_info.p, h->pb.p, h->o_i.p, h->o_j.p, h->o_meas.p, h->o_info.p,
                   h->Oii.p, h->Ojj.p, h->Oij.p, h->obi.p, h->obj.p, B.c, B.pb);
        SE2_HIP(hipGetLastError());
        return SE2GPU_OK;
    }
    if (fuse_lambda >= 0.0)
        SE2_LAUNCH(h->prof, st, "k_linearize", (k_linearize<true>), grid1((size_t)h->L * kGroup, kBlock), dim3(kBlock), 0,
                   h->cam, h->L, h->lm_ptr.p, h->e_kf.p, h->e_uv.p, h->e_info.p, B.pa, h->fixed.p, B.la, h->Hpl.p,
                   h->Hpp_e.p, h->bp_e.p, h->Hll.p, h->bl.p, fuse_lambda, h->Dinv.p, h->z.p, h->Dg.p, B.c, B.pb, B.lb, rec_twin(h));
    else
        SE2_LAUNCH(h->prof, st, "k_linearize0", (k_linearize<false>), grid1((size_t)h->L * kGroup, kBlock), dim3(kBlock), 0,
                   h->cam, h->L, h->lm_ptr.p, h->e_kf.p, h->e_uv.p, h->e_info.p, B.pa, h->fixed.p, B.la, h->Hpl.p,
                   h->Hpp_e.p, h->bp_e.p, h->Hll.p, h->bl.p, 0.0, h->Dinv.p, h->z.p, h->Dg.p, B.c, B.pb, B.lb, rec_twin(h));
    SE2_HIP(hipGetLastError());
    return SE2GPU_OK;
}

int ba_pose_blocks(se2gpu_ba* h, const double* poses, bool ctl = false, bool odometry_only = false) {
    hipStream_t st = h->stream;
    if (h->O) {
        if (ctl)
            SE2_LAUNCH(h->prof, st, "k_odometry", k_odometry, grid1(h->O, 64), dim3(64), 0, h->O, h->o_i.p, h->o_j.p,
                       h->o_meas.p, h->o_info.p, h->poses_a.p, h->fixed.p, h->Oii.p, h->Ojj.p, h->Oij.p, h->obi.p, h->obj.p,
                       (const BaCtl*)h->ctl.p, (const double*)h->poses_b.p);
        else
            SE2_LAUNCH(h->prof, st, "k_odometry", k_odometry, grid1(h->O, 64), dim3(64), 0, h->O, h->o_i.p, h->o_j.p,
                       h->o_meas.p, h->o_info.p, poses, h->fixed.p, h->Oii.p, h->Ojj.p, h->Oij.p, h->obi.p, h->obj.p,
                       (const BaCtl*)nullptr, (const double*)nullptr);
    }
    if (!odometry_only)
        SE2_LAUNCH(h->prof, st, "k_pose_reduce", k_pose_reduce, grid1((size_t)h->P * 64, kBlock), dim3(kBlock), 0, h->P,
                   h->pose_ptr.p, h->pose_edges.p, h->Hpp_e.p, h->bp_e.p, h->podo_ptr.p, h->podo_item.p, h->Oii.p,
                   h->Ojj.p, h->obi.p, h->obj.p, h->Hpp.p, h->bp.p);
    SE2_HIP(hipGetLastError());
    return SE2GPU_OK;
}

int ba_reduce(se2gpu_ba* h, double lambda, int schur, bool ctl = false) {
    hipStream_t st = h->stream;
    double* S = h->red;
    const Bufs B = bufs(h, ctl);
    if (h->model) {
        const double* pinfo = h->model == 2 ? h->ph.p : h->prior_info.p;
        if (schur && h->model == 1)
            SE2_LAUNCH(h->prof, st, "k3_schur_lm", k3_schur_lm, grid1((size_t)h->L * kGroup, kBlock), dim3(kBlock), 0, h->L,
                       lambda, h->lm_ptr.p, h->Hll.p, h->bl.p, h->Hpl.p, h->Hpp_e.p, h->bp_e.p, h->Dinv.p, h->z.p, h->Y.p,
                       h->Dg.p, B.c, schur == 2 ? 0 : 1);
        SE2_LAUNCH(h->prof, st, "k3_reduce2", k3_reduce2, dim3(((h->P + 1 + 7) & ~7) + ((h->nwg_off + 7) & ~7)), dim3(kBlock), 0,
                   h->P, h->ld, h->nwg_off, lambda, h->grp.p, h->blk_a.p, h->blk_b.p, h->pair_i.p, h->pair_j.p, h->blk_odo.p,
                   h->Y.p, h->Hpl.p, h->Dg.p, h->fixed.p, h->pose_ptr.p, h->pose_edges.p, h->podo_ptr.p, h->podo_item.p,
                   h->prior_has.p, pinfo, h->pb.p, h->Oii.p, h->Ojj.p, h->Oij.p, h->obi.p, h->obj.p, S, h->bp.p, B.c,
                   &h->ctl.p->epoch);
        SE2_HIP(hipGetLastError());
        return SE2GPU_OK;
    }
    if (schur) SE2_CHECK(ba_linearize(h, lambda, ctl));
    SE2_LAUNCH(h->prof, st, "k_reduce2", k_reduce2, dim3(((h->P + 1 + 7) & ~7) + ((h->nwg_off + 7) & ~7)), dim3(kBlock), 0, h->P, h->ld, h->nwg_off,
               lambda, h->root, h->grp.p, h->blk_a.p, h->blk_b.p, h->pair_i.p, h->pair_j.p, h->blk_odo.p,
               h->Hpl.p, h->Dg.p, h->fixed.p, h->pose_ptr.p, h->pose_edges.p,
               h->podo_ptr.p, h->podo_item.p, h->o_i.p, h->o_j.p, h->o_meas.p, h->o_info.p, B.pa, S, h->bp.p, B.c, B.pb,
               &h->ctl.p->epoch, (const int*)h->pose_off.p, h->nsys, (const double*)rec_twin(h).W, (const double*)rec_twin(h).Dg);
    if (h->O && h->odo_fallback) {
        SE2_LAUNCH(h->prof, st, "k_odometry", k_odometry, grid1(h->O, 64), dim3(64), 0, h->O, h->o_i.p, h->o_j.p,
                   h->o_meas.p, h->o_info.p, h->poses, h->fixed.p, h->Oii.p, h->Ojj.p, h->Oij.p, h->obi.p, h->obj.p,
                   (const BaCtl*)nullptr, (const double*)nullptr);
        SE2_LAUNCH(h->prof, st, "k_reduce_odo", k_reduce_odo, grid1((size_t)h->O * 9, 256), dim3(256), 0, h->O, h->ld,
                   h->o_i.p, h->o_j.p, h->Oij.p, S, (const int*)h->pose_off.p);
    }
    SE2_HIP(hipGetLastError());
    return SE2GPU_OK;
}

int ba_allreduce(se2gpu_ba* h, double* ptr, size_t count) {
    if (!h->allreduce) return SE2GPU_OK;
    h->prof.begin(h->stream);
    const int rc = h->allreduce(ptr, count, (void*)h->stream, h->ar_user);
    h->prof.end(h->stream, count > 4096 ? "allreduce_system" : "allreduce_small");
    SE2_REQUIRE(rc == 0, SE2GPU_ERR_HIP, "all-reduce callback failed with %d", rc);
    return SE2GPU_OK;
}

__host__ __device__ inline size_t tri_row_off(int r) {
    const size_t q = (size_t)(r / kNB), rem = (size_t)(r % kNB);
    return kNB * (kNB * q * (q + 1) / 2 + rem * (q + 1));
}
__global__ __launch_bounds__(256) void k_tri_pack(const double* __restrict__ A, int ld, int rows, double* __restrict__ packed,
                                                   int unpack, double* __restrict__ Aout) {
    const int r = blockIdx.x;
// ... 154 lines not shown
    SE2_HIP(hipGetLastError());
    return SE2GPU_OK;
}

int ba_lambda_init(se2gpu_ba* h) {
    hipStream_t st = h->stream;
    if (h->model) {
        SE2_LAUNCH(h->prof, st, "k3_pose_diag", k3_pose_diag, grid1((size_t)h->P * 64, kBlock), dim3(kBlock), 0, h->P,
                   h->pose_ptr.p, h->pose_edges.p, h->Hpp_e.p, h->fixed.p, h->prior_has.p,
                   h->model == 2 ? h->ph.p : h->prior_info.p, h->podo_ptr.p, h->podo_item.p, h->Oii.p, h->Ojj.p, h->diag3.p);
        SE2_LAUNCH(h->prof, st, "k_maxdiag", k_maxdiag, dim3(1), dim3(1024), 0, h->L, h->Hll.p, h->P, h->diag3.p,
                   h->fixed.p, h->scal.p, 6, 0, h->ctl.p);
        SE2_HIP(hipGetLastError());
        return SE2GPU_OK;
    }
    const bool sharded = h->allreduce && h->world > 1;
    const size_t nd = 3 * (size_t)h->P;
    if (!sharded) {
        SE2_CHECK(ba_pose_blocks(h, h->poses, true, true));
        const int nP = (h->P + kBlock / 64 - 1) / (kBlock / 64), nL = (h->L + kL0PerBlock - 1) / kL0PerBlock;
        SE2_LAUNCH(h->prof, st, "k_lambda0", k_lambda0, dim3(nP + nL), dim3(kBlock), 0, h->P, h->pose_ptr.p, h->pose_edges.p,
                   h->Hpp_e.p, h->bp_e.p, h->podo_ptr.p, h->podo_item.p, h->Oii.p, h->Ojj.p, h->obi.p, h->obj.p, h->Hpp.p,
                   h->bp.p, h->fixed.p, h->L, h->Hll.p, h->l0_acc.p, h->scal.p, h->ctl.p);
        SE2_HIP(hipGetLastError());
        return SE2GPU_OK;
    }
    SE2_CHECK(ba_pose_blocks(h, h->poses, true));
    SE2_LAUNCH(h->prof, st, "k_extract_diag", k_extract_diag, grid1((size_t)h->P * 3, 256), dim3(256), 0, h->P,
               h->Hpp.p, h->diag3.p);
    if (sharded) {
        SE2_HIP(hipMemcpyAsync(h->red, h->diag3.p, nd * 8, hipMemcpyDeviceToDevice, st));
        SE2_CHECK(ba_allreduce(h, h->red, nd));
        SE2_HIP(hipMemcpyAsync(h->diag3.p, h->red, nd * 8, hipMemcpyDeviceToDevice, st));
    }
    SE2_LAUNCH(h->prof, st, "k_maxdiag", k_maxdiag, dim3(1), dim3(1024), 0, h->L, h->Hll.p, h->P, h->diag3.p,
               h->fixed.p, h->scal.p, 3, 0, (BaCtl*)nullptr);
    if (sharded) {
        SE2_REQUIRE(h->world <= 1024, SE2GPU_ERR_INVALID, "world size %d > 1024", h->world);
        hipLaunchKernelGGL(k_fill_slots, dim3(1), dim3(1024), 0, st, h->red, h->scal.p, h->rank, h->world);
        SE2_CHECK(ba_allreduce(h, h->red, (size_t)h->world));
        hipLaunchKernelGGL(k_set_lambda, dim3(1), dim3(1), 0, st, h->ctl.p, h->red, h->world);
    } else {
        hipLaunchKernelGGL(k_set_lambda, dim3(1), dim3(1), 0, st, h->ctl.p, h->scal.p, 1);
    }
    SE2_HIP(hipGetLastError());
    return SE2GPU_OK;
}

int ba_enqueue_trial(se2gpu_ba* h, bool first, int know_retry, bool notify, double seq) {
    hipStream_t st = h->stream;
    const bool lm = h->run_mode == SE2GPU_BA_LM;
    const bool sharded = h->allreduce != nullptr;
    double* scal = h->red + (size_t)h->ld * h->ld;
    const Bufs B = bufs(h, true);
    auto evaluate = [&](bool step, bool note) -> int {
        if (h->model == 2) {
            if (step)
                SE2_LAUNCH(h->prof, st, "k4_oplus", k4_oplus, grid1(h->P, 64), dim3(64), 0, h->P, B.pa, h->fixed.p, h->xp.p, B.pb, B.c);
            SE2_LAUNCH(h->prof, st, "k4_finalize", k4_finalize, dim3(1), dim3(1024), 0, h->P, h->pg_edges, B.pa, B.pb, h->fixed.p,
                       h->xp.p, h->bp.p, h->prior_has.p, h->prior_meas.p, h->prior_info.p, h->pe_i.p, h->pe_j.p, h->pe_meas.p,
                       h->pe_info.p, scal, h->d_mail, seq, h->ctl.p, step ? 1 : 0, note ? 1 : 0, (const volatile int*)h->d_stop,
                       (double*)nullptr);
            SE2_HIP(hipGetLastError());
            return SE2GPU_OK;
        }
        if (h->model) {
            if (step)
                SE2_LAUNCH(h->prof, st, "k3_oplus", k3_oplus, grid1(h->P, 64), dim3(64), 0, h->P, B.pa, h->fixed.p, h->xp.p, B.pb, B.c);
            SE2_LAUNCH(h->prof, st, "k3_update", k3_update, grid1((size_t)h->L * kGroup, kBlock), dim3(kBlock), 0, h->cam3, h->L,
                       0.0, h->lm_ptr.p, h->e_kf.p, h->e_uv.p, h->e_info.p, B.pa, B.pb, B.la, h->xp.p, h->z.p, h->Y.p, h->bl.p,
                       B.lb, h->part.p, B.c, step ? 1 : 0, (double*)nullptr);
            SE2_LAUNCH(h->prof, st, "k3_finalize", k3_finalize, dim3(1), dim3(1024), 0, h->L ? h->nparts : 0, h->part.p, h->P,
                       B.pa, B.pb, h->fixed.p, h->xp.p, h->bp.p, h->prior_has.p, h->prior_meas.p, h->prior_info.p, h->O,
                       h->o_i.p, h->o_j.p, h->o_meas.p, h->o_info.p, scal, h->d_mail, seq, h->ctl.p, step ? 1 : 0, note ? 1 : 0,
                       (const volatile int*)h->d_stop);
            SE2_HIP(hipGetLastError());
            return SE2GPU_OK;
        }
        const dim3 ug = grid1((size_t)h->L * kGroup, kBlock);
        if (!sharded) {
            const bool lin = step && h->run_spec;
            FinArgs fin{1, (int)ug.x, h->P, h->O, h->root, step ? 1 : 0, 1, note ? 1 : 0, h->fixed.p, h->xp.p, h->bp.p, B.pa,
                        B.pb, h->o_i.p, h->o_j.p, h->o_meas.p, h->o_info.p, scal, h->d_mail, seq, h->ctl.p,
                        (const volatile int*)h->d_stop, h->fin_counter.p, lin ? 1 : 0};
            if (lin)
                SE2_LAUNCH(h->prof, st, "k_update_lin", k_update<true>, dim3(ug.x + 1), dim3(kBlock), 0, h->cam, h->L, 0.0, h->lm_ptr.p,
                           h->e_kf.p, h->e_uv.p, h->e_info.p, B.pa, h->fixed.p, B.la, (const double*)h->xp.p,
                           h->z.p, (const double*)h->Hpl.p, h->bl.p, B.lb, h->part.p, B.c, B.pb, fin, (const double*)h->Dinv.p,
                           SpecArgs{{rec_own(h), rec_twin(h)}, h->Hpp_e.p, h->bp_e.p});
            else
                SE2_LAUNCH(h->prof, st, "k_update", k_update<false>, dim3(ug.x + 1), dim3(kBlock), 0, h->cam, h->L, 0.0, h->lm_ptr.p,
                           h->e_kf.p, h->e_uv.p, h->e_info.p, B.pa, h->fixed.p, B.la, step ? h->xp.p : (const double*)nullptr,
                           h->z.p, (const double*)h->Hpl.p, h->bl.p, B.lb, h->part.p, B.c, B.pb, fin, (const double*)h->Dinv.p, SpecArgs{});
            SE2_HIP(hipGetLastError());
            return SE2GPU_OK;
        }
        SE2_LAUNCH(h->prof, st, "k_update", k_update<false>, ug, dim3(kBlock), 0, h->cam, h->L,
                   0.0, h->lm_ptr.p, h->e_kf.p, h->e_uv.p, h->e_info.p, B.pa, h->fixed.p, B.la,
                   step ? h->xp.p : (const double*)nullptr, h->z.p, (const double*)h->Hpl.p, h->bl.p, B.lb, h->part.p, B.c, B.pb, FinArgs{},
                   (const double*)h->Dinv.p, SpecArgs{});
        SE2_LAUNCH(h->prof, st, "k_finalize", k_finalize, dim3(1), dim3(1024), 0, h->L ? h->nparts : 0, h->part.p, h->P,
                   0.0, B.pa, h->fixed.p, h->xp.p, h->bp.p, B.pb, h->O, h->o_i.p, h->o_j.p, h->o_meas.p,
                   h->o_info.p, h->root, scal, h->d_mail, seq, h->ctl.p, step ? 1 : 0, sharded ? 0 : 1, note ? 1 : 0,
                   (const volatile int*)h->d_stop);
        if (sharded) {
            SE2_CHECK(ba_allreduce(h, scal, 4));
            hipLaunchKernelGGL(k_lm_decide, dim3(1), dim3(256), 0, st, h->ctl.p, scal, step ? 1 : 0, note ? 1 : 0,
                               h->d_mail, seq, (const volatile int*)h->d_stop);
        }
        SE2_HIP(hipGetLastError());
        return SE2GPU_OK;
    };
    if (first) {
        SE2_CHECK(evaluate(false, false));
        if (lm) {
            SE2_CHECK(ba_linearize(h, -1.0, true));
            SE2_CHECK(ba_lambda_init(h));
            SE2_CHECK(ba_reduce(h, 0.0, 3, true));
        } else {
            SE2_CHECK(ba_linearize(h, 0.0, true));
            SE2_CHECK(ba_reduce(h, 0.0, 0, true));
        }
    } else {
        if (know_retry != 1) SE2_CHECK(ba_linearize(h, 0.0, true));
        SE2_CHECK(ba_reduce(h, 0.0, !lm ? 0 : know_retry == 0 ? 0 : know_retry == 1 ? 3 : (h->model ? 2 : 0), true));
    }
    SE2_CHECK(ba_allreduce_system(h));
    SE2_CHECK(ba_solve(h, true));
    SE2_CHECK(evaluate(true, notify));
    return SE2GPU_OK;
}


template <typename... A>
struct Packed {
    int nblk;
    std::tuple<A...> args;
};
template <auto Body, int BS, typename... A>
__global__ __launch_bounds__(BS) void k_batched(const Packed<A...>* __restrict__ p) {
    const Packed<A...>& x = p[blockIdx.y];
    if ((int)blockIdx.x >= x.nblk) return;
    std::apply([&](const A&... a) { Body(blockIdx.x, a...); }, x.args);
}
template <auto Body, int BS, typename... A>
__global__ __launch_bounds__(BS) void k_batched_xcd(const Packed<A...>* __restrict__ p) {
    const unsigned nb = gridDim.x, nw8 = gridDim.y & ~7u;
    unsigned w = blockIdx.y, bx = blockIdx.x;
    if (w < nw8) {
        const unsigned lin = w * nb + bx, k = lin >> 3;
        w = 8 * (k / nb) + (lin & 7);
        bx = k % nb;
    }
    const Packed<A...>& x = p[w];
    if ((int)bx >= x.nblk) return;
    std::apply([&](const A&... a) { Body(bx, a...); }, x.args);
}

struct BatchArena {
    std::vector<uint8_t> host;
    DevBuf<uint8_t> dev;
    size_t add(const void* src, size_t bytes) {
        const size_t off = (host.size() + 255) & ~(size_t)255;
        host.resize(off + bytes);
        std::memcpy(host.data() + off, src, bytes);
        return off;
    }
};
template <auto Body, int BS>
struct BatchKernel;
template <typename... A, void (*Body)(unsigned, A...), int BS>
struct BatchKernel<Body, BS> {
    using P = Packed<std::remove_cv_t<A>...>;
    std::vector<P> packs;
    size_t off = 0;
    int maxblk = 0;
    void add(int nblk, A... a) {
        packs.push_back(P{nblk, std::tuple<std::remove_cv_t<A>...>(a...)});
        maxblk = std::max(maxblk, nblk);
    }
    void commit(BatchArena& ar) { off = ar.add(packs.data(), packs.size() * sizeof(P)); }
    void launch(const BatchArena& ar, hipStream_t st, int block = BS, size_t shmem = 0) const {
        if (packs.empty() || maxblk <= 0) return;
        hipLaunchKernelGGL((k_batched<Body, BS, std::remove_cv_t<A>...>), dim3((unsigned)maxblk, (unsigned)packs.size()), dim3(block),
                           shmem, st, reinterpret_cast<const P*>(ar.dev.p + off));
    }
    void launch_xcd(const BatchArena& ar, hipStream_t st) const {
        if (packs.empty() || maxblk <= 0) return;
        static const bool eight = [] {
            int dev = 0, n = 0;
            return hipGetDevice(&dev) == hipSuccess && hipDeviceGetAttribute(&n, hipDeviceAttributeNumberOfXccs, dev) == hipSuccess && n == 8;
        }();
        if (!eight) { launch(ar, st); return; }
        hipLaunchKernelGGL((k_batched_xcd<Body, BS, std::remove_cv_t<A>...>), dim3((unsigned)((maxblk + 7) & ~7), (unsigned)packs.size()),
                           dim3(BS), 0, st, reinterpret_cast<const P*>(ar.dev.p + off));
    }
    static const void* kernel() { return (const void*)k_batched<Body, BS, std::remove_cv_t<A>...>; }
};

struct BatchPlan {
    std::vector<se2gpu_ba*> hs;
    std::vector<unsigned long> serials;
    std::vector<hipStream_t> streams;
    int iters = -1, mode = -1;
    BatchArena arena;
    hipStream_t stream = nullptr;
    BatchKernel<d_ctl_init, 64> ctl_init;
// ... 122 lines not shown
                            fail, h->chol_trace.p, (const BaCtl*)h->ctl.p, h->xp.p, (unsigned long long*)nullptr, h->chol_head.p, h->chol_ntask);
        }
    }
    bp.ctl_init.commit(bp.arena); bp.eval0.commit(bp.arena); bp.step.commit(bp.arena); bp.step_notify.commit(bp.arena);
    bp.lin0.commit(bp.arena); bp.lin.commit(bp.arena); bp.odo.commit(bp.arena); bp.pose_reduce.commit(bp.arena);
    bp.maxdiag.commit(bp.arena); bp.reduce2.commit(bp.arena);
    bp.chol.commit(bp.arena); bp.chol_v.commit(bp.arena);
    SE2_CHECK(bp.arena.dev.reserve(bp.arena.host.size()));
    SE2_HIP(hipMemcpyAsync(bp.arena.dev.p, bp.arena.host.data(), bp.arena.host.size(), hipMemcpyHostToDevice, bp.stream));
    bp.events.resize(count);
    return SE2GPU_OK;
}

int ba_batch_slot(const BatchPlan& bp, bool first, bool notify) {
    hipStream_t st = bp.stream;
    const BatchArena& ar = bp.arena;
    const bool lm = bp.mode == SE2GPU_BA_LM;
    if (first) {
        bp.eval0.launch(ar, st);
        if (lm) {
            bp.lin0.launch(ar, st);
            bp.odo.launch(ar, st);
            bp.pose_reduce.launch(ar, st);
            bp.maxdiag.launch(ar, st);
            bp.lin.launch(ar, st);
        } else {
            bp.lin.launch(ar, st);
        }
    } else {
        bp.lin.launch(ar, st);
    }
    bp.reduce2.launch_xcd(ar, st);
    if (bp.verify) bp.chol_v.launch(ar, st);
    else bp.chol.launch(ar, st);
    (notify ? bp.step_notify : bp.step).launch(ar, st);
    SE2_HIP(hipGetLastError());
    return SE2GPU_OK;
}

}

static int ba_fetch_estimates(se2gpu_ba* h);

extern "C" {

namespace {
constexpr size_t kPoolMax = 4;
static std::mutex g_ba_pool_mu;
static std::vector<se2gpu_ba*> g_ba_pool;
static bool ba_pool_enabled() {
    static const bool on = env_flag("SE2GPU_BA_POOL", true);
    return on;
}
}

int se2gpu_ba_create(se2gpu_ba** out) {
    SE2_REQUIRE(out, SE2GPU_ERR_INVALID, "ba_create: out is NULL");
    SE2_REQUIRE(have_device(), SE2GPU_ERR_NO_DEVICE, "no HIP device visible (libse2gpu has no CPU fallback)");
    int dev = 0;
    SE2_HIP(hipGetDevice(&dev));
    {
        std::lock_guard<std::mutex> lk(g_ba_pool_mu);
        for (size_t i = 0; i < g_ba_pool.size(); ++i)
            if (g_ba_pool[i]->device == dev) {
                *out = g_ba_pool[i];
                g_ba_pool.erase(g_ba_pool.begin() + (ptrdiff_t)i);
                return SE2GPU_OK;
            }
    }
    se2gpu_ba* h = new se2gpu_ba;
    h->device = dev;
    if (hipStreamCreateWithFlags(&h->own_stream, hipStreamNonBlocking) != hipSuccess) {
        delete h;
        set_error("hipStreamCreate failed");
        return SE2GPU_ERR_HIP;
    }
    h->stream = h->own_stream;
    *out = h;
    return SE2GPU_OK;
}

void se2gpu_ba_destroy(se2gpu_ba* h) {
    if (!h) return;
    if (h->join_event) { (void)hipEventSynchronize(h->join_event); h->join_event = nullptr; h->join_stream = nullptr; }
    if (ba_pool_enabled()) {
        (void)hipStreamSynchronize(h->stream);
        if (h->own_stream != h->stream) (void)hipStreamSynchronize(h->own_stream);
        (void)se2gpu_ba_clear(h);
        h->own_pending = false;
        h->have_tbc = false;
        const double I3[9] = {1, 0, 0, 0, 1, 0, 0, 0, 1};
        std::memcpy(h->Rbc, I3, sizeof(I3));
        h->tbc[0] = h->tbc[1] = h->tbc[2] = 0;
        h->stream = h->own_stream;
        h->prof.enabled = false;
        h->prof.reset();
        h->allreduce = nullptr; h->ar_user = nullptr; h->comm = nullptr; h->ar_buffer = nullptr;
        h->red = nullptr;
        h->root = 1; h->rank = 0; h->world = 1;
        std::lock_guard<std::mutex> lk(g_ba_pool_mu);
        if (g_ba_pool.size() < kPoolMax) {
            g_ba_pool.push_back(h);
            return;
        }
    }
    delete h;
}

int se2gpu_ba_clear(se2gpu_ba* h) {
    SE2_REQUIRE(h, SE2GPU_ERR_INVALID, "ba handle is NULL");
    h->pose_of_id.clear(); h->lm_of_id.clear(); h->pose_ids.clear(); h->lm_ids.clear();
    h->h_poses.clear(); h->h_lms.clear(); h->h_fixed.clear(); h->odo.clear();
    h->he_kf.clear(); h->he_lm.clear(); h->he_uv.clear(); h->he_info.clear();
    h->huber_delta = 0; h->huber_mixed = false;
    h->bulk_E = 0; h->bulk_kf = h->bulk_lm = nullptr; h->bulk_uv = h->bulk_info = nullptr;
    h->model = 0; h->D = 3; h->ps = 3;
    h->h_prior_has.clear(); h->h_prior_meas.clear(); h->h_prior_info.clear(); h->odo3.clear(); h->edge_perm.clear();
    h->pg_edges = 0; h->pg_perm.clear();
    h->lg_active = false;
    h->lg_lc.clear(); h->lg_lw.clear(); h->lg_sigma2.clear(); h->lg_Rcw.clear(); h->lg_twb.clear();
    h->have_cam = false;
    h->initialized = false;
    h->est_valid = false;
    return SE2GPU_OK;
}

int se2gpu_ba_reserve(int P, int L, int E) {
    SE2_REQUIRE(P >= 2 && L >= 1 && E >= L, SE2GPU_ERR_INVALID, "ba_reserve: need P >= 2, L >= 1, E >= L (got %d, %d, %d)", P, L, E);
    SE2_REQUIRE(ba_pool_enabled(), SE2GPU_ERR_STATE, "ba_reserve: the handle pool is disabled (SE2GPU_BA_POOL=0)");
    E = (int)std::min<long long>(E, (long long)L * P);
    se2gpu_ba* h = nullptr;
    SE2_CHECK(se2gpu_ba_create(&h));
    struct Guard { se2gpu_ba* h; ~Guard() { se2gpu_ba_destroy(h); } } guard{h};
    const double fx = 400, cx = 320, cy = 240;
    SE2_CHECK(se2gpu_ba_add_cam(h, fx, cx, cy));
    for (int i = 0; i < P; ++i) SE2_CHECK(se2gpu_ba_add_vertex_se2(h, i, 100.0 * i, 0.0, 0.0, i == 0));
    const double info3[9] = {1, 0, 0, 0, 1, 0, 0, 0, 1};
    for (int i = 0; i + 1 < P; ++i) {
        const double meas[3] = {100.0, 0.0, 0.0};
        SE2_CHECK(se2gpu_ba_add_edge_se2(h, i, i + 1, meas, info3));
    }
    std::vector<double> lm(3 * (size_t)L);
    for (int l = 0; l < L; ++l) {
        lm[3 * (size_t)l] = 50.0 * P + 37.0 * (l % 41) - 700.0;
        lm[3 * (size_t)l + 1] = 23.0 * (l % 53) - 600.0;
        lm[3 * (size_t)l + 2] = 3000.0 + 11.0 * (l % 97);
        SE2_CHECK(se2gpu_ba_add_vertex_xyz(h, P + l, &lm[3 * (size_t)l], 1, 0));
    }
    const double info2[4] = {1, 0, 0, 1};
    const int base = E / L, extra = E % L;
    for (int l = 0; l < L; ++l) {
        const int k = base + (l < extra ? 1 : 0);
        for (int j = 0; j < k; ++j) {
            const int kf = (int)(((long long)l * 7 + j) % P);
            const double xc = lm[3 * (size_t)l] - 100.0 * kf, yc = lm[3 * (size_t)l + 1], zc = lm[3 * (size_t)l + 2];
            const double uv[2] = {fx * xc / zc + cx, fx * yc / zc + cy};
            SE2_CHECK(se2gpu_ba_add_edge_se2xyz(h, kf, P + l, uv, info2, 2.4477));
        }
    }
    SE2_CHECK(se2gpu_ba_initialize(h));
    se2gpu_ba_stats st;
    SE2_CHECK(se2gpu_ba_optimize(h, 1, SE2GPU_BA_LM, nullptr, 0, &st));
    if (ba_env_speculate()) SE2_CHECK(ba_reserve_twin(h));
    double xyt[3];
    SE2_CHECK(se2gpu_ba_get_se2(h, 0, xyt));
    return SE2GPU_OK;
// ... 501 lines not shown
            for (int r = 0; r < D; ++r) {
                const int ra = h->h_pose_off[a] + r;
                if (bs) bs[D * a + r] = full[(size_t)ns * ld + ra];
                if (S)
                    for (int b = 0; b < h->P; ++b)
                        for (int c = 0; c < D; ++c) S[(size_t)(D * a + r) * n + D * b + c] = full[(size_t)ra * ld + h->h_pose_off[b] + c];
            }
        return SE2GPU_OK;
    }
    if (S)
        SE2_HIP(hipMemcpy2D(S, (size_t)n * 8, h->red, (size_t)h->ld * 8, (size_t)n * 8, n, hipMemcpyDeviceToHost));
    if (bs) SE2_HIP(hipMemcpy(bs, h->red + (size_t)n * h->ld, (size_t)n * 8, hipMemcpyDeviceToHost));
    return SE2GPU_OK;
}

int se2gpu_ba_debug_solve_plan_tile(int P, int D, const uint8_t* pattern, int allow_nd, int tile, int* nsys, int* nbc, int* depth, int* ntask,
                                    int* ndep, int32_t* pose_off, int32_t* tasks4, int task_cap, int32_t* deps, int dep_cap) {
    SE2_REQUIRE(P > 0 && (D == 3 || D == 6) && (tile == 32 || tile == 64) && nsys && nbc && depth && ntask && ndep, SE2GPU_ERR_INVALID, "debug_solve_plan_tile: bad argument");
    SolvePlan sp;
    solve_plan_choose(P, D, pattern, allow_nd != 0, sp, false, tile);
    *nsys = sp.nsys; *nbc = sp.nbc; *depth = sp.depth; *ntask = (int)sp.tasks.size(); *ndep = (int)sp.deps.size();
    if (pose_off) std::memcpy(pose_off, sp.pose_off.data(), (size_t)P * 4);
    if (tasks4) {
        SE2_REQUIRE(task_cap >= (int)sp.tasks.size(), SE2GPU_ERR_CAPACITY, "debug_solve_plan_tile: %zu tasks", sp.tasks.size());
        std::memcpy(tasks4, sp.tasks.data(), sp.tasks.size() * sizeof(int4));
    }
    if (deps) {
        SE2_REQUIRE(dep_cap >= (int)sp.deps.size(), SE2GPU_ERR_CAPACITY, "debug_solve_plan_tile: %zu dependency entries", sp.deps.size());
        std::memcpy(deps, sp.deps.data(), sp.deps.size() * 4);
    }
    return SE2GPU_OK;
}

int se2gpu_ba_debug_solve_plan(int P, int D, const uint8_t* pattern, int allow_nd, int* nsys, int* nbc, int* depth, int* ntask,
                               int* ndep, int32_t* pose_off, int32_t* tasks4, int task_cap, int32_t* deps, int dep_cap) {
    SE2_REQUIRE(P > 0 && (D == 3 || D == 6) && nsys && nbc && depth && ntask && ndep, SE2GPU_ERR_INVALID, "debug_solve_plan: bad argument");
    SolvePlan sp;
    solve_plan_choose(P, D, pattern, allow_nd != 0, sp);
    *nsys = sp.nsys; *nbc = sp.nbc; *depth = sp.depth; *ntask = (int)sp.tasks.size(); *ndep = (int)sp.deps.size();
    if (pose_off) std::memcpy(pose_off, sp.pose_off.data(), (size_t)P * 4);
    if (tasks4) {
        SE2_REQUIRE(task_cap >= (int)sp.tasks.size(), SE2GPU_ERR_CAPACITY, "debug_solve_plan: %zu tasks", sp.tasks.size());
        std::memcpy(tasks4, sp.tasks.data(), sp.tasks.size() * sizeof(int4));
    }
    if (deps) {
        SE2_REQUIRE(dep_cap >= (int)sp.deps.size(), SE2GPU_ERR_CAPACITY, "debug_solve_plan: %zu dependency entries", sp.deps.size());
        std::memcpy(deps, sp.deps.data(), sp.deps.size() * 4);
    }
    return SE2GPU_OK;
}

int se2gpu_ba_debug_chol_verify(se2gpu_ba* h, unsigned long long* counts2, unsigned long long* records, int cap) {
    SE2_REQUIRE(h && h->initialized && h->chol_vfy.p, SE2GPU_ERR_STATE, "the handle does not verify its hand-offs (SE2GPU_BA_CHOL_VERIFY=1)");
    SE2_CHECK(ba_join(h));
    SE2_HIP(hipStreamSynchronize(h->stream));
    unsigned long long head[8];
    SE2_HIP(hipMemcpy(head, h->chol_vfy.p, sizeof(head), hipMemcpyDeviceToHost));
    counts2[0] = head[0]; counts2[1] = head[1];
    const int nrec = (int)std::min<unsigned long long>(std::min<unsigned long long>(head[0], kVfyRecords), (unsigned long long)std::max(cap, 0));
    if (nrec && records) SE2_HIP(hipMemcpy(records, h->chol_vfy.p + 8, (size_t)nrec * 8 * sizeof(unsigned long long), hipMemcpyDeviceToHost));
    return SE2GPU_OK;
}

int se2gpu_ba_debug_pool_sizes(int out2[2]) {
    SE2_REQUIRE(out2, SE2GPU_ERR_INVALID, "debug_pool_sizes: NULL argument");
    { LeasePool<PlanSet>& p = LeasePool<PlanSet>::get(); std::lock_guard<std::mutex> g(p.mu); out2[0] = (int)p.idle.size(); }
    { LeasePool<ResetScratch>& p = LeasePool<ResetScratch>::get(); std::lock_guard<std::mutex> g(p.mu); out2[1] = (int)p.idle.size(); }
    return SE2GPU_OK;
}

int se2gpu_ba_debug_solver_path(const se2gpu_ba* h) {
    if (!h || !h->initialized) return -1;
    return h->host_solve ? 3 : h->chol_fallback ? 2 : h->chol_steps ? 1 : 0;
}

int se2gpu_ba_debug_linearize_counts(const se2gpu_ba* h, int* runs, int* skips, long long* twin_bytes) {
    SE2_REQUIRE(h && h->initialized, SE2GPU_ERR_STATE, "debug_linearize_counts before initialize");
    BaCtl c;
    std::memset(&c, 0, sizeof(c));
    if (h->h_mail && !h->run_active) std::memcpy(&c, (const void*)(h->h_mail + 8), sizeof(BaCtl));
    if (runs) *runs = c.lin_runs;
    if (skips) *skips = c.lin_skips;
    if (twin_bytes) *twin_bytes = (long long)(h->rec_twin.cap * sizeof(double));
    return SE2GPU_OK;
}

int se2gpu_ba_debug_solve(se2gpu_ba* h, double lambda, double* x, int* factor_ok) {
    SE2_REQUIRE(h && h->initialized && x, SE2GPU_ERR_STATE, "debug_solve before initialize");
    SE2_CHECK(ba_join(h));
    const int n = h->D * h->P;
    SE2_CHECK(ba_linearize(h, lambda));
    SE2_CHECK(ba_reduce(h, lambda, false));
    SE2_CHECK(ba_allreduce(h, h->red, (size_t)(h->nsys + 1) * h->ld));
    SE2_CHECK(ba_solve(h));
    SE2_HIP(hipStreamSynchronize(h->stream));
    SE2_HIP(hipMemcpy(x, h->xp.p, (size_t)n * 8, hipMemcpyDeviceToHost));
    double f = 0;
    SE2_HIP(hipMemcpy(&f, h->red + (size_t)h->ld * h->ld + 2, 8, hipMemcpyDeviceToHost));
    SE2_REQUIRE(f < 1e5, SE2GPU_ERR_HIP, "k_chol_tiles: a dependency spin timed out (2 s)");
    if (factor_ok) *factor_ok = !(f > 0.0);
    if (h->chol_trace.p && !h->chol_steps) {
        std::vector<long long> tr(16 * (size_t)h->chol_ntask);
        std::vector<int4> tk(h->chol_ntask);
        SE2_HIP(hipMemcpy(tr.data(), h->chol_trace.p, tr.size() * sizeof(long long), hipMemcpyDeviceToHost));
        SE2_HIP(hipMemcpy(tk.data(), h->chol_tasks.p, tk.size() * sizeof(int4), hipMemcpyDeviceToHost));
        int ndep = 0;
        for (const int4& t : tk) ndep = std::max(ndep, t.w);
        std::vector<int> dp((size_t)std::max(ndep, 1));
        if (ndep) SE2_HIP(hipMemcpy(dp.data(), h->chol_deps.p, (size_t)ndep * sizeof(int), hipMemcpyDeviceToHost));
        long long t0 = tr[0];
        for (int t = 0; t < h->chol_ntask; ++t) t0 = std::min(t0, tr[16 * (size_t)t]);
        for (int t = 0; t < h->chol_ntask; ++t) {
            std::fprintf(stderr, "choltrace %d %d %d %d %d", t, tk[t].x & 0xffff, tk[t].x >> 16, tk[t].y,
                         tk[t].w > tk[t].z ? dp[tk[t].w - 1] : -1);
            for (int q = 0; q < 6; ++q) std::fprintf(stderr, " %lld", tr[16 * (size_t)t + q] ? tr[16 * (size_t)t + q] - t0 : -1);
            std::fprintf(stderr, " %lld %lld", tr[16 * (size_t)t + 6], tr[16 * (size_t)t + 7] ? tr[16 * (size_t)t + 7] - t0 : -1);
            for (int q = 8; q < 16; ++q) std::fprintf(stderr, " %lld", tr[16 * (size_t)t + q] ? tr[16 * (size_t)t + q] - t0 : -1);
            std::fprintf(stderr, "\n");
        }
    }
    return SE2GPU_OK;
}

namespace {

bool ba_env_sync() {
    static const bool on = env_flag("SE2GPU_BA_SYNC", false);
    return on;
}

int ba_run_prologue(se2gpu_ba* h, hipStream_t st, hipEvent_t* ev, int iters, int mode, bool sync, const volatile uint8_t* stop_flag) {
    SE2_CHECK(ba_join(h, st, ev));
    h->est_valid = false;
    h->run_mode = mode;
    h->run_iters = iters;
    h->run_enqueued = 0;
    h->run_sync = sync;
    h->run_spec = false;
    h->run_active = true;
    *h->h_stop = (stop_flag && *stop_flag) ? 1 : 0;
    return SE2GPU_OK;
}

int ba_run_begin(se2gpu_ba* h, int iters, int mode, const volatile uint8_t* stop_flag, int verbose) {
    SE2_REQUIRE(h && h->initialized, SE2GPU_ERR_STATE, "optimize before initialize");
    SE2_REQUIRE(mode == SE2GPU_BA_LM || mode == SE2GPU_BA_GN, SE2GPU_ERR_INVALID, "unknown mode %d", mode);
    SE2_REQUIRE(h->d_mail, SE2GPU_ERR_STATE, "SE2GPU_BA_MAILBOX=0 is no longer supported: the LM controller posts its state "
                                              "through the mapped mailbox");
    const bool sync = ba_env_sync() || h->prof.enabled || verbose || h->odo_fallback || h->host_solve;
    SE2_CHECK(ba_run_prologue(h, h->stream, nullptr, iters, mode, sync, stop_flag));
    h->run_spec = ba_env_speculate() && h->model == 0 && !h->allreduce && !h->comm && h->L > 0 && iters > 1;
    if (h->run_spec) SE2_CHECK(ba_reserve_twin(h));
    const int n0 = h->run_sync ? 1 : std::max(iters, 1);
    auto enqueue_all = [&]() -> int {
        hipLaunchKernelGGL(k_ctl_init, dim3(1), dim3(64), 0, h->stream, h->ctl.p, iters, mode);
        SE2_HIP(hipGetLastError());
        for (int k = 0; k < n0; ++k) SE2_CHECK(ba_enqueue_trial(h, k == 0, h->run_sync ? 0 : -1, k == n0 - 1, 0.0));
        return SE2GPU_OK;
    };
    static const bool graphs_on = env_flag("SE2GPU_BA_GRAPH", true);
    const bool graphable = graphs_on && !h->run_sync && !h->allreduce && !h->comm && iters > 0;
    se2gpu_ba::GraphSlot* slot = nullptr;
    if (graphable) {
        for (auto& g : h->graphs)
            if (g.iters == iters && g.mode == mode) slot = &g;
        if (!slot) {
            slot = &h->graphs[0];
            for (auto& g : h->graphs)
                if (g.stamp < slot->stamp) slot = &g;
            if (slot->exec) (void)hipGraphExecDestroy(slot->exec);
            *slot = se2gpu_ba::GraphSlot{};
            slot->iters = iters;
            slot->mode = mode;
            slot->stamp = ++h->graph_clock;
            SE2_CHECK(enqueue_all());
        } else if (slot->exec) {
            slot->stamp = ++h->graph_clock;
            SE2_HIP(hipGraphLaunch(slot->exec, h->stream));
        } else {
            slot->stamp = ++h->graph_clock;
            hipGraph_t g = nullptr;
            SE2_HIP(hipStreamBeginCapture(h->stream, hipStreamCaptureModeThreadLocal));
            const int rc = enqueue_all();
            const hipError_t ce = hipStreamEndCapture(h->stream, &g);
            SE2_CHECK(rc);
            SE2_HIP(ce);
            const hipError_t ie = hipGraphInstantiate(&slot->exec, g, nullptr, nullptr, 0);
            (void)hipGraphDestroy(g);
            SE2_HIP(ie);
            SE2_HIP(hipGraphLaunch(slot->exec, h->stream));
        }
    } else {
        SE2_CHECK(enqueue_all());
    }
    h->dev_seq += n0;
    h->run_seq = h->dev_seq;
    h->run_enqueued = n0;
    return SE2GPU_OK;
}

int ba_run_step(se2gpu_ba* h, bool wait, const volatile uint8_t* stop_flag, int verbose, int* finished) {
    *finished = 0;
    if (stop_flag && *stop_flag) *h->h_stop = 1;
    const double first = h->run_seq - h->run_enqueued;
    if (wait) SE2_CHECK(ba_wait_seq(h, kMailSeq, h->run_seq, first, &h, 1, stop_flag, 30, "the LM controller never reported back"));
    else if (!ba_mail_at(h, kMailSeq, h->run_seq, first)) return SE2GPU_OK;
    std::atomic_thread_fence(std::memory_order_acquire);
    BaCtl c;
    std::memcpy(&c, (const void*)(h->h_mail + 8), sizeof(BaCtl));
    if (c.error && !h->chol_steps) {
        std::fprintf(stderr, "se2gpu_ba: k_chol_tiles timed out; continuing with k_chol_step\n");
        h->chol_steps = h->chol_fallback = true;
        h->drop_graphs();
        SE2_HIP(hipStreamSynchronize(h->stream));
        hipLaunchKernelGGL(k_ctl_clear_error, dim3(1), dim3(1), 0, h->stream, h->ctl.p);
        c.error = 0;
        c.done = 0;
        h->run_enqueued = 0;
        ((volatile double*)h->h_mail)[kMailSeq] = 0.0;
    }
    SE2_REQUIRE(!c.error, SE2GPU_ERR_HIP, "k_chol_step: the factorisation reported a time-out");
    if (verbose)
        fprintf(stderr, "se2gpu_ba: it %d trial %d chi2 %.9g rho %.3g lambda %.6g%s\n", c.it, c.qmax, c.current_chi, c.rho,
                c.lambda, c.retry ? " (rejected)" : "");
    if (h->run_sync)
        if ((h->poses == h->poses_b.p) != (c.sel != 0)) { std::swap(h->poses, h->poses_t); std::swap(h->lms, h->lms_t); }
    if (c.done) {
        *finished = 1;
        return SE2GPU_OK;
    }
    const int more = h->run_sync ? 1 : std::max(1, c.iters - c.it);
    for (int k = 0; k < more; ++k) {
        SE2_CHECK(ba_enqueue_trial(h, false, h->run_sync ? (c.retry ? 1 : 0) : -1, k == more - 1, 0.0));
        h->dev_seq += 1;
        h->run_seq = h->dev_seq;
        ++h->run_enqueued;
    }
    return SE2GPU_OK;
}

int ba_run_finish(se2gpu_ba* h, se2gpu_ba_stats* stats) {
    h->own_pending = false;
    BaCtl c;
    std::memcpy(&c, (const void*)(h->h_mail + 8), sizeof(BaCtl));
    h->run_active = false;
    if ((h->poses == h->poses_b.p) != (c.sel != 0)) { std::swap(h->poses, h->poses_t); std::swap(h->lms, h->lms_t); }
    if (stats) {
        se2gpu_ba_stats s;
        std::memset(&s, 0, sizeof(s));
        s.iterations = c.it;
        s.trials = c.trials;
        s.terminated = c.terminated;
        s.stopped = c.stopped;
        s.chi2_init = c.chi2_init;
        s.chi2_final = c.chi2_final;
        s.lambda_final = c.lambda;
        std::memcpy(s.chi2_hist, c.chi2_hist, sizeof(s.chi2_hist));
        std::memcpy(s.lambda_hist, c.lambda_hist, sizeof(s.lambda_hist));
        std::memcpy(s.trials_hist, c.trials_hist, sizeof(s.trials_hist));
        *stats = s;
    }
    return SE2GPU_OK;
}

struct BatchExit {
    se2gpu_ba* const* hs;
    int count;
    ~BatchExit() {
        for (int i = 0; i < count; ++i)
            if (hs[i]->run_active) {
                (void)hipStreamSynchronize(hs[i]->stream);
                hs[i]->run_active = false;
            }
    }
};

struct ResidentScratch {
    PinBuf<WindowArgs> host;
    DevBuf<WindowArgs> dev;
    PinBuf<Window3Args> host3;
    DevBuf<Window3Args> dev3;
    DevBuf<long long> stamps;
    std::vector<hipEvent_t> events;
};
int ba_resident_threads(const se2gpu_ba* h, size_t* lds) {
    int nfree = 0;
    for (int p = 0; p < h->P; ++p) nfree += h->h_fixed[p] ? 0 : 1;
    for (int t : {512, 256, 128}) {
        const size_t b = h->model == 1 ? ba_window3_lds_bytes(h->P, nfree, t) : ba_window_lds_bytes(h->P, nfree, t);
        if (b) { *lds = b; return t; }
    }
    return 0;
}
bool ba_resident_ok(const se2gpu_ba* h) {
    const size_t rec = h->model == 1 ? 28 : 44;
    return ba_batchable(h) && h->model <= 1 && !h->odo_self_loop && h->P > 0 && (int)h->h_fixed.size() == h->P && h->Hpl.p &&
           h->Hpl.cap * 8 >= (size_t)h->L * 16 + (size_t)h->E * rec + 16 && h->Dinv.p && h->Dinv.cap >= 6 * (size_t)h->L;
}
int ba_optimize_resident(se2gpu_ba** hs, int count, int iters, int mode, const volatile uint8_t* stop_flag,
                         se2gpu_ba_stats* stats, int* handled) {
    *handled = 0;
    const int env_on = env_int("SE2GPU_BA_RESIDENT", -1), env_min = env_int("SE2GPU_BA_RESIDENT_MIN", 96);
    if (env_on == 0 || (env_on != 1 && count < env_min)) return SE2GPU_OK;
    struct Item { int i, threads, model; size_t lds; };
    std::vector<Item> items((size_t)count);
    for (int i = 0; i < count; ++i) {
        if (!ba_resident_ok(hs[i])) return SE2GPU_OK;
        size_t b = 0;
        const int t = ba_resident_threads(hs[i], &b);
        if (!t) return SE2GPU_OK;
        if (t < 256 && env_on != 1) return SE2GPU_OK;
        items[(size_t)i] = Item{i, t, hs[i]->model, b};
    }
    std::stable_sort(items.begin(), items.end(), [&](const Item& a, const Item& b) {
        if (a.threads != b.threads) return a.threads > b.threads;
        if (a.model != b.model) return a.model > b.model;
        return hs[a.i]->E > hs[b.i]->E;
    });
    auto same_class = [&](int k0, int k1) { return items[(size_t)k0].threads == items[(size_t)k1].threads && items[(size_t)k0].model == items[(size_t)k1].model; };
    static std::mutex launch_mu;
    Lease<ResidentScratch> lease;
    ResidentScratch& rs = *lease.obj;
    SE2_CHECK(rs.host.reserve((size_t)count));
    SE2_CHECK(rs.dev.reserve((size_t)count));
    SE2_CHECK(rs.host3.reserve((size_t)count));
    SE2_CHECK(rs.dev3.reserve((size_t)count));
    static const bool trace = env_flag("SE2GPU_BA_RESIDENT_TRACE", false);
    if (trace) SE2_CHECK(rs.stamps.reserve(16 * (size_t)count));
    if (rs.events.size() < (size_t)count) rs.events.resize((size_t)count);
    std::vector<hipStream_t> class_streams;
    int threads = 0;
    size_t lds = 0;
    BatchExit exit_guard{hs, count};
    for (int k = 0; k < count; ++k) {
        const int i = items[(size_t)k].i;
        se2gpu_ba* h = hs[i];
        if (k == 0 || !same_class(k, k - 1)) class_streams.push_back(h->stream);
        SE2_CHECK(ba_run_prologue(h, class_streams.back(), &rs.events[(size_t)k], iters, mode, false, stop_flag));
        if (h->model == 1) {
            Window3Args& a = rs.host3.p[k];
            a.cam = h->cam3;
            a.P = h->P; a.L = h->L; a.E = h->E; a.O = h->O; a.iters = iters; a.mode = mode;
            a.lm_ptr = h->lm_ptr.p; a.e_kf = h->e_kf.p; a.e_uv = h->e_uv.p; a.e_info = h->e_info.p;
            a.poses_a = h->poses_a.p; a.poses_b = h->poses_b.p; a.lms_a = h->lms_a.p; a.lms_b = h->lms_b.p;
            a.fixed = h->fixed.p;
            a.prior_has = h->prior_has.p; a.prior_meas = h->prior_meas.p; a.prior_info = h->prior_info.p;
            a.o_i = h->o_i.p; a.o_j = h->o_j.p; a.o_meas = h->o_meas.p; a.o_info = h->o_info.p;
            a.ctl = h->ctl.p;
            a.mail = h->d_mail;
            a.stop = h->d_stop;
            a.desc = reinterpret_cast<int4*>(h->Hpl.p);
            a.ainv = h->Dinv.p;
            a.stamps = trace ? rs.stamps.p + 16 * (size_t)k : nullptr;
            continue;
        }
// ... 376 lines not shown
```

se2lam_amd/csrc/ba_device.h:

```cpp
#pragma once
#include <hip/hip_runtime.h>

#include <cmath>

#include "../../include/se2gpu.h"

namespace se2gpu {
namespace badev {

constexpr int kGroup = 8;
constexpr int kBlock = 256;
constexpr double kPi = 3.14159265358979323846;

struct CamDev {
    double fx, cx, cy;
    double Rcb[9];
    double tcb[3];
    double huber;
};

constexpr int kMailSeq = 4;
struct BaCtl {
    double lambda, ni, current_chi, rho;
    double chi2_init, chi2_final;
    int it, qmax, trials, iters;
    int done, terminated, stopped, retry;
    int sel;
    int mode, error, pad;
    double chi2_hist[64], lambda_hist[64];
    int trials_hist[64];
    int rec_sel, rec_valid, lin_runs, lin_skips;
    double seq;
    unsigned epoch;
    unsigned pad2;
};

__host__ __device__ inline double normalize_theta(double theta) {
    if (theta >= -kPi && theta < kPi) return theta;
    double multiplier = floor(theta / (2 * kPi));
    theta = theta - multiplier * 2 * kPi;
    if (theta >= kPi) theta -= 2 * kPi;
    if (theta < -kPi) theta += 2 * kPi;
    return theta;
}

template <bool JAC>
__device__ inline void se2xyz(const CamDev& cam, double px, double py, double pth, double lx, double ly, double lz,
                              double u, double v, double& e0, double& e1, double* Jp, double* Jl) {
    double s, c;
    sincos(pth, &s, &c);
    const double dx = lx - px, dy = ly - py;
    double R[9];
#pragma unroll
    for (int i = 0; i < 3; ++i) {
        R[i * 3 + 0] = cam.Rcb[i * 3 + 0] * c - cam.Rcb[i * 3 + 1] * s;
        R[i * 3 + 1] = cam.Rcb[i * 3 + 0] * s + cam.Rcb[i * 3 + 1] * c;
        R[i * 3 + 2] = cam.Rcb[i * 3 + 2];
    }
    const double X = R[0] * dx + R[1] * dy + R[2] * lz + cam.tcb[0];
    const double Y = R[3] * dx + R[4] * dy + R[5] * lz + cam.tcb[1];
    const double Z = R[6] * dx + R[7] * dy + R[8] * lz + cam.tcb[2];
    const double zi = 1.0 / Z;
    e0 = cam.fx * X * zi + cam.cx - u;
    e1 = cam.fx * Y * zi + cam.cy - v;
    if (JAC) {
        const double zi2 = zi * zi;
        const double j00 = cam.fx * zi, j02 = -cam.fx * X * zi2, j12 = -cam.fx * Y * zi2;
#pragma unroll
        for (int k = 0; k < 3; ++k) {
            Jl[k] = j00 * R[k] + j02 * R[6 + k];
            Jl[3 + k] = j00 * R[3 + k] + j12 * R[6 + k];
        }
        Jp[0] = -Jl[0]; Jp[1] = -Jl[1]; Jp[2] = Jl[0] * dy - Jl[1] * dx;
        Jp[3] = -Jl[3]; Jp[4] = -Jl[4]; Jp[5] = Jl[3] * dy - Jl[4] * dx;
    }
}

__device__ inline void huber(double e2, double delta, double& rho0, double& rho1) {
    const double dsqr = delta * delta;
    if (e2 <= dsqr) {
        rho0 = e2; rho1 = 1.0;
    } else {
        const double sq = sqrt(e2);
        rho0 = 2 * sq * delta - dsqr;
        rho1 = delta / sq;
    }
}

template <int CTRL>
__device__ __forceinline__ double dpp_partner(double v) {
    const long long b = __double_as_longlong(v);
    int lo = (int)(b & 0xffffffffll), hi = (int)(b >> 32);
    lo = __builtin_amdgcn_mov_dpp(lo, CTRL, 0xf, 0xf, true);
    hi = __builtin_amdgcn_mov_dpp(hi, CTRL, 0xf, 0xf, true);
    return __longlong_as_double(((long long)hi << 32) | (unsigned int)lo);
}
__device__ inline double group_sum(double v) {
    static_assert(kGroup == 8, "three butterfly steps");
    v += dpp_partner<0xB1>(v);
    v += dpp_partner<0x4E>(v);
    v += dpp_partner<0x141>(v);
    return v;
}

__device__ inline double wave_sum(double v) {
    v += dpp_partner<0xB1>(v);
    v += dpp_partner<0x4E>(v);
    v += dpp_partner<0x141>(v);
    v += dpp_partner<0x140>(v);
    v += __shfl_xor(v, 16);
    v += __shfl_xor(v, 32);
    return v;
}

__device__ inline void chol_inv3(const double h[6], double lambda, double a[6]) {
    const double m00 = h[0] + lambda, m10 = h[1], m20 = h[2], m11 = h[3] + lambda, m21 = h[4], m22 = h[5] + lambda;
    const double floor_ = 1e-30 * (m00 + m11 + m22);
// ... 91 lines not shown
```

se2lam_amd/optimizer.py:

```python
from __future__ import annotations

import ctypes as C
import os

import numpy as np

from . import capi

LM, GN = 0, 1


def _stats_dict(st):
    n = min(st.iterations, 64)
    return dict(iterations=st.iterations, trials=st.trials, terminated=bool(st.terminated),
                stopped=bool(st.stopped), chi2_init=st.chi2_init, chi2_final=st.chi2_final,
                lambda_final=st.lambda_final, chi2_hist=list(st.chi2_hist[:n]),
                lambda_hist=list(st.lambda_hist[:n]), trials_hist=list(st.trials_hist[:n]))


def _no_fallback(h):
    if capi.lib().se2gpu_ba_debug_solver_path(h) == 2 and os.environ.get("SE2GPU_BA_CHOL_FAULT") != "1":
        raise RuntimeError("se2gpu_ba: k_chol_tiles timed out and the handle fell back to k_chol_step")


# ... 3 lines not shown
    capi.check(capi.lib().se2gpu_ba_reset_estimates_batch(hs, n))


def optimize_batch(optimizers, iterations: int, mode: int = 0, stop=None):
    n = len(optimizers)
    hs = (C.c_void_p * n)(*[o._h for o in optimizers])
    st = (capi.BaStats * n)()
    sp = stop.ctypes.data_as(C.POINTER(C.c_uint8)) if stop is not None else None
    capi.check(capi.lib().se2gpu_ba_optimize_batch(hs, n, int(iterations), int(mode), sp, st))
    resident = capi.lib().se2gpu_ba_last_batch_path() == 2
    for o, s in zip(optimizers, st):
        o._stats, o._stats_raw = None, s
        if not resident:
            _no_fallback(o._h)
    return [s.iterations for s in st]


class SlamOptimizer:

    def __init__(self):
        self._h = C.c_void_p()
        capi.check(capi.lib().se2gpu_ba_create(C.byref(self._h)))
        self._stop = None
        self._verbose = False
        self._cb = None
        self._keep = []
        self._stats = None
        self._stats_raw = None

    @property
    def stats(self):
        if self._stats is None and self._stats_raw is not None:
            self._stats = _stats_dict(self._stats_raw)
        return self._stats

    @stats.setter
    def stats(self, value):
        self._stats, self._stats_raw = value, None

    def stat(self, name: str):
        return getattr(self._stats_raw, name) if self._stats_raw is not None else self.stats[name]

    def setVerbose(self, v: bool):
        self._verbose = bool(v)

    def setForceStopFlag(self, flag: np.ndarray | None):
        self._stop = flag

    def clear(self):
        capi.check(capi.lib().se2gpu_ba_clear(self._h))

    def clearParameters(self):
        """g2o drops the camera parameters here, not in clear(); this harness re-adds the camera with every load()"""

    def initializeOptimization(self, level: int = 0):
        assert level == 0
        capi.check(capi.lib().se2gpu_ba_initialize(self._h))

    def optimize(self, iterations: int, mode: int = LM) -> int:
        st = capi.BaStats()
        stop = self._stop.ctypes.data_as(C.POINTER(C.c_uint8)) if self._stop is not None else None
        capi.check(capi.lib().se2gpu_ba_optimize(self._h, int(iterations), int(mode), stop, int(self._verbose),
                                                 C.byref(st)))
        self.stats = _stats_dict(st)
        _no_fallback(self._h)
        return st.iterations

    def exchange_doubles(self) -> int:
        return int(capi.lib().se2gpu_ba_exchange_doubles_h(self._h))

    def chol_verify(self):
        counts = np.zeros(2, np.uint64)
        rec = np.zeros((64, 8), np.uint64)
        capi.check(capi.lib().se2gpu_ba_debug_chol_verify(self._h, counts.ctypes.data, rec.ctypes.data, 64))
        return int(counts[0]), int(counts[1]), rec[:min(int(counts[0]), 64)]

    def solver_path(self) -> int:
        return int(capi.lib().se2gpu_ba_debug_solver_path(self._h))

    def linearize_counts(self):
        runs, skips, twin = C.c_int(0), C.c_int(0), C.c_longlong(0)
        capi.check(capi.lib().se2gpu_ba_debug_linearize_counts(self._h, C.byref(runs), C.byref(skips), C.byref(twin)))
        return int(runs.value), int(skips.value), int(twin.value)

    def activeRobustChi2(self) -> float:
        v = capi.lib().se2gpu_ba_chi2(self._h)
        if v < 0:
            capi.check(capi.ERR_STATE)
        return float(v)

    def load(self, g):
        l = capi.lib()
        capi.check(l.se2gpu_ba_add_cam(self._h, g.fx, g.cx, g.cy))
        R = np.ascontiguousarray(g.Rbc, np.float64).reshape(-1)
        t = np.ascontiguousarray(g.tbc, np.float64).reshape(-1)
        capi.check(l.se2gpu_ba_set_Tbc(self._h, capi.pd(R), capi.pd(t)))
        a = [np.ascontiguousarray(g.poses, np.float64), np.ascontiguousarray(g.fixed, np.uint8),
             np.ascontiguousarray(g.lms, np.float64), np.ascontiguousarray(g.e_kf, np.int32),
             np.ascontiguousarray(g.e_lm, np.int32), np.ascontiguousarray(g.e_uv, np.float64),
             np.ascontiguousarray(g.e_info, np.float64), np.ascontiguousarray(g.o_i, np.int32),
             np.ascontiguousarray(g.o_j, np.int32), np.ascontiguousarray(g.o_meas, np.float64),
             np.ascontiguousarray(g.o_info, np.float64)]
        P32, PU8 = C.POINTER(C.c_int32), C.POINTER(C.c_uint8)
        capi.check(l.se2gpu_ba_load(self._h, g.P, g.L, g.E, g.O, capi.pd(a[0]), a[1].ctypes.data_as(PU8),
                                    capi.pd(a[2]), a[3].ctypes.data_as(P32), a[4].ctypes.data_as(P32),
                                    capi.pd(a[5]), capi.pd(a[6]), a[7].ctypes.data_as(P32),
                                    a[8].ctypes.data_as(P32), capi.pd(a[9]), capi.pd(a[10]), float(g.huber)))
        self._shape = (g.P, g.L)
        self._keep = a

    def estimates(self):
        P, L = self._shape
        poses = np.zeros((P, getattr(self, "_pose_dim", 3)))
        lms = np.zeros((max(L, 1), 3))
        capi.check(capi.lib().se2gpu_ba_get_all(self._h, capi.pd(poses), capi.pd(lms)))
        return poses, lms[:L]

    def reset_estimates(self):
        capi.check(capi.lib().se2gpu_ba_reset_estimates(self._h))

    def reduced_system(self, lam: float):
        P, _ = self._shape
        n = (6 if getattr(self, "_pose_dim", 3) == 12 else 3) * P
        S = np.zeros((n, n))
        bs = np.zeros(n)
        capi.check(capi.lib().se2gpu_ba_debug_reduced_system(self._h, float(lam), capi.pd(S), capi.pd(bs)))
        return S, bs

    def solve(self, lam: float):
        P, _ = self._shape
        x = np.zeros(3 * P)
        ok = C.c_int(0)
        capi.check(capi.lib().se2gpu_ba_debug_solve(self._h, float(lam), capi.pd(x), C.byref(ok)))
        return x, bool(ok.value)

    def set_shard(self, rank: int, world: int):
        capi.check(capi.lib().se2gpu_ba_set_shard(self._h, rank, world))

    def set_allreduce(self, fn, buffer_ptr=None):
        def _tramp(ptr, count, stream, user):
            try:
                fn(ptr, count, stream)
                return 0
            except Exception as exc:
                print(f"se2lam_amd: all-reduce callback failed: {exc!r}")
                return 1
        self._cb = capi.ALLREDUCE_FN(_tramp)
        capi.check(capi.lib().se2gpu_ba_set_allreduce(self._h, self._cb, None, buffer_ptr))

    def set_comm(self, comm):
        capi.check(capi.lib().se2gpu_ba_set_comm(self._h, comm))

    def reduce_buffer_doubles(self, P: int) -> int:
        return int(capi.lib().se2gpu_ba_reduce_buffer_doubles(self._h, P))

    def set_stream(self, stream_ptr):
        capi.check(capi.lib().se2gpu_ba_set_stream(self._h, stream_ptr))

    def stream(self):
        return capi.lib().se2gpu_ba_stream(self._h)

    def profile(self, enable: bool):
        capi.check(capi.lib().se2gpu_ba_profile(self._h, int(enable)))

    def profile_report(self):
        out = {}
# ... 229 lines not shown
```

Baseline: 6932 iters/s.

## Repair mis-speculated linearization in-launch with extra spinning workgroups

Adds R extra workgroups to the fused update/linearize kernel. They spin until the finisher publishes a verdict, and when the speculative linearization record missed they relinearize on the accepted state inside the same launch. This removes the separate k_linearize launch on retry paths. In exchange it adds spin-wait workgroups that hold CU slots, agent-scope loads and stores, a timeout error path, a process-wide occupancy budget, and graph slots keyed by the repair count.

```diff
diff --git a/include/se2gpu.h b/include/se2gpu.h
--- a/include/se2gpu.h
+++ b/include/se2gpu.h
@@ -194,6 +194,7 @@
 int se2gpu_ba_debug_solve(se2gpu_ba* h, double lambda, double* x, int* factor_ok);
 int se2gpu_ba_debug_solver_path(const se2gpu_ba* h);
 int se2gpu_ba_debug_linearize_counts(const se2gpu_ba* h, int* runs, int* skips, long long* twin_bytes);
+int se2gpu_ba_debug_repair_workgroups(const se2gpu_ba* h, int* last_run, int* process_waiters, int* lin_launches);
 int se2gpu_ba_debug_pool_sizes(int out2[2]);
 int se2gpu_ba_debug_chol_verify(se2gpu_ba* h, unsigned long long* counts2, unsigned long long* records, int cap);
 int se2gpu_ba_debug_solve_plan(int P, int D, const uint8_t* pattern, int allow_nd, int* nsys, int* nbc, int* depth, int* ntask,
diff --git a/se2lam_amd/capi.py b/se2lam_amd/capi.py
--- a/se2lam_amd/capi.py
+++ b/se2lam_amd/capi.py
@@ -141,6 +141,7 @@
     "se2gpu_ba_debug_solve": (_I, [_VP, _D, _PD, C.POINTER(C.c_int)]),
     "se2gpu_ba_debug_solver_path": (_I, [_VP]),
     "se2gpu_ba_debug_linearize_counts": (_I, [_VP, C.POINTER(C.c_int), C.POINTER(C.c_int), C.POINTER(C.c_longlong)]),
+    "se2gpu_ba_debug_repair_workgroups": (_I, [_VP, C.POINTER(C.c_int), C.POINTER(C.c_int), C.POINTER(C.c_int)]),
     "se2gpu_ba_debug_chol_verify": (_I, [_VP, _VP, _VP, _I]),
     "se2gpu_ba_debug_pool_sizes": (_I, [_VP]),
     "se2gpu_ba_debug_solve_plan": (_I, [_I, _I, _VP, _I, _VP, _VP, _VP, _VP, _VP, _VP, _VP, _I, _VP, _I]),
diff --git a/se2lam_amd/csrc/ba.hip b/se2lam_amd/csrc/ba.hip
--- a/se2lam_amd/csrc/ba.hip
+++ b/se2lam_amd/csrc/ba.hip
@@ -945,6 +945,8 @@
 __device__ inline void store_agent(double* p, d2_t v) {
     asm volatile("global_store_dwordx4 %0, %1, off sc1\n\ts_nop 1" : : "v"(p), "v"(v) : "memory");
 }
+__device__ inline double load_agent1(const double* p) { return __hip_atomic_load(p, __ATOMIC_RELAXED, __HIP_MEMORY_SCOPE_AGENT); }
+__device__ inline void store_agent1(double* p, double v) { __hip_atomic_store(p, v, __ATOMIC_RELAXED, __HIP_MEMORY_SCOPE_AGENT); }
 #define SE2_WAIT_VM6(a, b, c, d, e, f) \
     asm volatile("s_waitcnt vmcnt(0)" : "+v"(a), "+v"(b), "+v"(c), "+v"(d), "+v"(e), "+v"(f) : : "memory")
 
@@ -1338,13 +1340,104 @@
     const volatile int* stop;
     unsigned* counter;
     int spec;
+    int repair;
 };
 __device__ void finish_trial(const FinArgs& fin, const double* part, double lambda, double* fsp);
 
 struct SpecArgs {
     RecSet set[2];
     double *Hpp_e, *bp_e;
+    double *Hpp_r, *bp_r;
 };
+
+constexpr unsigned kVerdictEpoch = 0x1fffffffu;
+struct RepairArgs {
+    const int *lm_ptr, *e_kf;
+    const double *e_uv, *e_info, *poses, *lms;
+    const uint8_t* fixed;
+    RecSet wr;
+    double *Hpp_e, *bp_e;
+    double lambda;
+    int L, nblk, R, pad;
+};
+__device__ __forceinline__ unsigned long long uniform64(unsigned long long b) {
+    return (unsigned long long)(unsigned)__builtin_amdgcn_readfirstlane((int)(b & 0xffffffffull)) |
+           (unsigned long long)(unsigned)__builtin_amdgcn_readfirstlane((int)(b >> 32)) << 32;
+}
+template <typename T>
+__device__ __forceinline__ T* uniform_ptr(T* p) { return reinterpret_cast<T*>(uniform64(reinterpret_cast<unsigned long long>(p))); }
+__device__ __forceinline__ void repair_trial(const unsigned bx, const CamDev& cam, int L, const int* __restrict__ lm_ptr,
+                                             const int* __restrict__ e_kf, const double* __restrict__ e_uv,
+                                             const double* __restrict__ e_info, const double* poses_a, const double* poses_b,
+                                             const uint8_t* __restrict__ fixed, const double* lms_a, const double* lms_b,
+                                             BaCtl* ctl, int nblk, int R, RecSet set0, RecSet set1,
+                                             double* Hpp_e, double* bp_e, double* keep) {
+    __shared__ unsigned verdict_s;
+    __shared__ RepairArgs args_s;
+    if (threadIdx.x == 0) {
+        const unsigned want = ctl->epoch & kVerdictEpoch;
+        unsigned v = __hip_atomic_load(&ctl->verdict, __ATOMIC_RELAXED, __HIP_MEMORY_SCOPE_AGENT);
+        const long long t0 = wall_clock64();
+        while ((v >> 3) != want) {
+            __builtin_amdgcn_s_sleep(16);
+            if (wall_clock64() - t0 > 200000000ll) {
+                __hip_atomic_store(&ctl->error, 2, __ATOMIC_RELAXED, __HIP_MEMORY_SCOPE_AGENT);
+                __hip_atomic_store(&ctl->done, 1, __ATOMIC_RELAXED, __HIP_MEMORY_SCOPE_AGENT);
+                v = 0;
+                break;
+            }
+            v = __hip_atomic_load(&ctl->verdict, __ATOMIC_RELAXED, __HIP_MEMORY_SCOPE_AGENT);
+        }
+        verdict_s = v;
+        if (v & 1u) {
+            const bool b = (v & 4u) != 0, alt = (v & 2u) != 0;
+            args_s = RepairArgs{lm_ptr, e_kf, e_uv, e_info, b ? poses_b : poses_a, b ? lms_b : lms_a, fixed,
+                                RecSet{alt ? set1.W : set0.W, alt ? set1.Dg : set0.Dg, alt ? set1.Hll : set0.Hll, alt ? set1.bl : set0.bl,
+                                       alt ? set1.Ainv : set0.Ainv, alt ? set1.zeta : set0.zeta},
+                                Hpp_e, bp_e, load_agent1(&ctl->lambda), L, nblk, R, 0};
+        }
+    }
+    __syncthreads();
+    if (!(verdict_s & 1u)) return;
+    int blk = (int)bx - nblk - 1;
+    for (;;) {
+        asm volatile("" : "+s"(blk) : : "memory");
+        const RepairArgs* as = &args_s;
+        const int* lmp = uniform_ptr(as->lm_ptr);
+        const int* ekf = uniform_ptr(as->e_kf);
+        const double* euv = uniform_ptr(as->e_uv);
+        const double* einfo = uniform_ptr(as->e_info);
+        const double* poses = uniform_ptr(as->poses);
+        const double* lms = uniform_ptr(as->lms);
+        const uint8_t* fx = uniform_ptr(as->fixed);
+        const RecSet wr{uniform_ptr(as->wr.W), uniform_ptr(as->wr.Dg), uniform_ptr(as->wr.Hll), uniform_ptr(as->wr.bl),
+                        uniform_ptr(as->wr.Ainv), uniform_ptr(as->wr.zeta)};
+        double* hppe = uniform_ptr(as->Hpp_e);
+        double* bpe_ = uniform_ptr(as->bp_e);
+        const double lambda = __longlong_as_double((long long)uniform64((unsigned long long)__double_as_longlong(as->lambda)));
+        const int nL = __builtin_amdgcn_readfirstlane(as->L);
+        const int gid = blk * kBlock + threadIdx.x;
+        const int l = gid / kGroup, sub = gid % kGroup;
+        double hll[6] = {0, 0, 0, 0, 0, 0}, b[3] = {0, 0, 0};
+        int beg = 0, end = 0;
+        if (l < nL) {
+            const double lx = load_agent1(lms + 3 * (size_t)l), ly = load_agent1(lms + 3 * (size_t)l + 1),
+                         lz = load_agent1(lms + 3 * (size_t)l + 2);
+            beg = lmp[l];
+            end = lmp[l + 1];
+            for (int e = beg + sub; e < end; e += kGroup) {
+                const int kf = ekf[e];
+                double hpl[9], hpp[6], bpe[3], r0;
+                lin_edge(cam, load_agent1(poses + 3 * kf), load_agent1(poses + 3 * kf + 1), load_agent1(poses + 3 * kf + 2), lx, ly, lz,
+                         euv[2 * e], euv[2 * e + 1], einfo[3 * e], einfo[3 * e + 1], einfo[3 * e + 2], !fx[kf], hll, b, hpl, hpp, bpe, r0);
+                lin_park<true>(e == beg + sub, e, hpl, hpp, bpe, keep, wr.W, hppe, bpe_);
+            }
+        }
+        lin_landmark<true>(l, sub, beg, end, nL, hll, b, lambda, keep, wr.W, hppe, bpe_, wr.Hll, wr.bl, wr.Ainv, wr.zeta, wr.Dg);
+        blk += __builtin_amdgcn_readfirstlane(as->R);
+        if (blk >= __builtin_amdgcn_readfirstlane(as->nblk)) break;
+    }
+}
 
 template <bool LIN>
 __device__ __forceinline__ void d_update(const unsigned bx, CamDev cam, int L, double lambda, const int* __restrict__ lm_ptr,
@@ -1359,8 +1452,11 @@
                                                     FinArgs fin, const double* __restrict__ Ainv, SpecArgs sp) {
     __shared__ double lds[LIN ? (kBlock / 64) * kWaveLds : 3 * 1024];
     static_assert((kBlock / 64) * kWaveLds >= 3 * 1024, "the finisher's pose stage");
-    if (fin.enabled && (int)bx == fin.nblk) {
-        finish_trial(fin, part, lambda, lds);
+    if (fin.enabled && (int)bx >= fin.nblk) {
+        if ((int)bx == fin.nblk) finish_trial(fin, part, lambda, lds);
+        else if constexpr (LIN)
+            repair_trial(bx, cam, L, lm_ptr, e_kf, e_uv, e_info, poses, poses_b, fixed, lms, lms_trial, fin.ctl, fin.nblk, fin.repair,
+                         sp.set[0], sp.set[1], sp.Hpp_r, sp.bp_r, lds);
         return;
     }
     const int gid = bx * kBlock + threadIdx.x;
@@ -1370,11 +1466,14 @@
         beg = lm_ptr[l];
         end = lm_ptr[l + 1];
     }
+    const double* pz = poses;
+    const double* lz = lms;
+    double* lt = lms_trial;
     if (ctl) {
         if (ctl->done) return;
         if (ctl->sel) {
-            const double* t = lms; lms = lms_trial; lms_trial = const_cast<double*>(t);
-            poses = poses_b;
+            lz = lms_trial; lt = const_cast<double*>(lms);
+            pz = poses_b;
         }
         lambda = ctl->lambda;
     }
@@ -1417,7 +1516,7 @@
 #pragma unroll
     for (int k = 0; k < KS; ++k) {
         const int kf = ekf[k];
-        epose[k][0] = poses[3 * kf]; epose[k][1] = poses[3 * kf + 1]; epose[k][2] = poses[3 * kf + 2];
+        epose[k][0] = pz[3 * kf]; epose[k][1] = pz[3 * kf + 1]; epose[k][2] = pz[3 * kf + 2];
         efix[k] = fixed[kf] != 0;
 #pragma unroll
         for (int i = 0; i < 3; ++i) ep[k][i] = step ? xp[3 * kf + i] : 0.0;
@@ -1426,7 +1525,7 @@
     if (l < L) {
 #pragma unroll
         for (int c = 0; c < 3; ++c) {
-            lw0[c] = lms[(size_t)l * 3 + c];
+            lw0[c] = lz[(size_t)l * 3 + c];
             if (step) { zz[c] = zeta[(size_t)l * 3 + c]; blv[c] = bl[(size_t)l * 3 + c]; }
         }
         if (step) {
@@ -1464,7 +1563,8 @@
         if (sub == 0 && step) {
 #pragma unroll
             for (int c = 0; c < 3; ++c) {
-                lms_trial[(size_t)l * 3 + c] = lw[c];
+                if (LIN) store_agent1(lt + (size_t)l * 3 + c, lw[c]);
+                else lt[(size_t)l * 3 + c] = lw[c];
                 scale += x[c] * (lambda * x[c] + blv[c]);
             }
         }
@@ -1495,7 +1595,7 @@
             const int kf = e_kf[e];
             double dp[3] = {0, 0, 0};
             if (step) { dp[0] = xp[3 * kf]; dp[1] = xp[3 * kf + 1]; dp[2] = xp[3 * kf + 2]; }
-            edge_chi(e, poses[3 * kf], poses[3 * kf + 1], poses[3 * kf + 2], fixed[kf] != 0, dp, e_uv[2 * e], e_uv[2 * e + 1],
+            edge_chi(e, pz[3 * kf], pz[3 * kf + 1], pz[3 * kf + 2], fixed[kf] != 0, dp, e_uv[2 * e], e_uv[2 * e + 1],
                      e_info[3 * e], e_info[3 * e + 1], e_info[3 * e + 2]);
         }
     }
@@ -1503,6 +1603,7 @@
     scale = wave_sum(scale);
     const int w = threadIdx.x / 64;
     if ((threadIdx.x & 63) == 0) { sm[0][w] = chi; sm[1][w] = scale; }
+    if (LIN) asm volatile("s_waitcnt vmcnt(0)" ::: "memory");
     __syncthreads();
     if (threadIdx.x == 0) {
         double c = 0, s = 0;
@@ -1573,6 +1674,8 @@
     double failflag = 0;
     if (ctl) {
         if (ctl->done) {
+            if (fin.repair && threadIdx.x == 0)
+                __hip_atomic_store(&ctl->verdict, (ctl->epoch & kVerdictEpoch) << 3, __ATOMIC_RELAXED, __HIP_MEMORY_SCOPE_AGENT);
             end_slot(ctl, mail, fin.notify != 0, threadIdx.x, blockDim.x, fin.step != 0);
             return;
         }
@@ -1593,9 +1696,12 @@
             if (fin.root) scale += d0 * (lambda * d0 + bp[3 * p]) + d1 * (lambda * d1 + bp[3 * p + 1]) + d2 * (lambda * d2 + bp[3 * p + 2]);
             else scale += d0 * bp[3 * p] + d1 * bp[3 * p + 1] + d2 * bp[3 * p + 2];
         }
-        if (step) { poses_trial[3 * p] = x; poses_trial[3 * p + 1] = y; poses_trial[3 * p + 2] = th; }
+        if (step && fin.repair) {
+            store_agent1(poses_trial + 3 * p, x); store_agent1(poses_trial + 3 * p + 1, y); store_agent1(poses_trial + 3 * p + 2, th);
+        } else if (step) { poses_trial[3 * p] = x; poses_trial[3 * p + 1] = y; poses_trial[3 * p + 2] = th; }
         if (p < 1024) { fsp[3 * p] = x; fsp[3 * p + 1] = y; fsp[3 * p + 2] = th; }
     }
+    if (fin.repair) asm volatile("s_waitcnt vmcnt(0)" ::: "memory");
     __syncthreads();
     for (int k = threadIdx.x; k < fin.O; k += blockDim.x) {
         const int i = fin.o_i[k], j = fin.o_j[k];
@@ -1655,6 +1761,13 @@
                 const double lambda_spec = lm_lambda_spec(ctl->lambda, ctl->mode);
                 lm_advance(ctl, sc, stopped != 0);
                 if (!ctl->error) lm_records_advance(ctl, speculated, sel0, lambda_spec);
+                if (fin.repair) {
+                    const unsigned miss = (ctl->done | ctl->rec_valid) ? 0u : 1u;
+                    store_agent1(&ctl->lambda, ctl->lambda);
+                    asm volatile("s_waitcnt vmcnt(0)" ::: "memory");
+                    __hip_atomic_store(&ctl->verdict, (ctl->epoch & kVerdictEpoch) << 3 | (unsigned)(ctl->sel & 1) << 2 | (unsigned)(ctl->rec_sel & 1) << 1 | miss,
+                                       __ATOMIC_RELAXED, __HIP_MEMORY_SCOPE_AGENT);
+                }
             }
             fpost = (ctl->done || fin.notify) && mail;
         } else if (mail && !ctl) {
@@ -2689,6 +2802,8 @@
     DevBuf<double> red_own, xp, part, scal, diag3, Rinv;
     DevBuf<double> rec_twin;
     bool run_spec = false;
+    int run_repair = 0, repair_held = 0, last_repair = 0;
+    int run_lin_launches = 0;
     DevBuf<double> red_packed;
     DevBuf<int4> chol_tasks;
     DevBuf<int> chol_deps;
@@ -2708,7 +2823,7 @@
     DevBuf<unsigned> fin_counter;
     DevBuf<unsigned long long> l0_acc;
     int chol_ntask = 0;
-    struct GraphSlot { int iters = -1, mode = -1; hipGraphExec_t exec = nullptr; unsigned long stamp = 0; };
+    struct GraphSlot { int iters = -1, mode = -1, repair = 0, lin_launches = 0; hipGraphExec_t exec = nullptr; unsigned long stamp = 0; };
     static constexpr int kGraphSlots = 3;
     GraphSlot graphs[kGraphSlots];
     unsigned long graph_clock = 0;
@@ -4035,6 +4150,40 @@
     static const bool on = env_flag("SE2GPU_BA_SPECULATE", true);
     return on;
 }
+bool ba_env_repair_inlaunch() {
+    static const bool on = env_flag("SE2GPU_BA_REPAIR_INLAUNCH", true);
+    return on;
+}
+int ba_update_lin_capacity() {
+    static const int capacity = [] {
+        int per_cu = 0, dev = 0;
+        hipDeviceProp_t pr{};
+        if (hipGetDevice(&dev) != hipSuccess || hipGetDeviceProperties(&pr, dev) != hipSuccess) return 0;
+        if (hipOccupancyMaxActiveBlocksPerMultiprocessor(&per_cu, reinterpret_cast<const void*>(&k_update<true>), kBlock, 0) != hipSuccess) return 0;
+        return per_cu * pr.multiProcessorCount;
+    }();
+    return capacity;
+}
+std::atomic<int> g_repair_waiters{0};
+void ba_repair_release(se2gpu_ba* h) {
+    if (h->repair_held) g_repair_waiters.fetch_sub(h->repair_held, std::memory_order_relaxed);
+    h->repair_held = 0;
+}
+int ba_repair_acquire(se2gpu_ba* h) {
+    ba_repair_release(h);
+    if (!ba_env_repair_inlaunch()) return 0;
+    const int capacity = ba_update_lin_capacity();
+    const int nblk = (int)grid1((size_t)h->L * kGroup, kBlock).x;
+    const int R = std::min(capacity - (nblk + 1), nblk);
+    if (R < 1 || 8 * R < nblk) return 0;
+    const int waiters = R + 1;
+    if (g_repair_waiters.fetch_add(waiters, std::memory_order_relaxed) + waiters > capacity / 2) {
+        g_repair_waiters.fetch_sub(waiters, std::memory_order_relaxed);
+        return 0;
+    }
+    h->repair_held = waiters;
+    return R;
+}
 RecSet rec_own(const se2gpu_ba* h) { return RecSet{h->Hpl.p, h->Dg.p, h->Hll.p, h->bl.p, h->Dinv.p, h->z.p}; }
 RecSet rec_twin(const se2gpu_ba* h) {
     if (!h->rec_twin.p || h->model) return RecSet{};
@@ -4049,7 +4198,11 @@
     r.zeta = p;
     return r;
 }
-int ba_reserve_twin(se2gpu_ba* h) { return h->rec_twin.reserve(21 * (size_t)h->E + 18 * (size_t)h->L + 6); }
+double* rec_park(const se2gpu_ba* h, bool bp) {
+    if (!h->rec_twin.p || h->model) return nullptr;
+    return h->rec_twin.p + 21 * (size_t)h->E + 18 * (size_t)h->L + 6 + (bp ? 6 * (size_t)h->E + 1 : 0);
+}
+int ba_reserve_twin(se2gpu_ba* h) { return h->rec_twin.reserve(30 * (size_t)h->E + 18 * (size_t)h->L + 8); }
 
 
 int ba_linearize(se2gpu_ba* h, double fuse_lambda, bool ctl = false) {
@@ -4077,6 +4230,7 @@
         SE2_HIP(hipGetLastError());
         return SE2GPU_OK;
     }
+    if (fuse_lambda >= 0.0) ++h->run_lin_launches;
     if (fuse_lambda >= 0.0)
         SE2_LAUNCH(h->prof, st, "k_linearize", (k_linearize<true>), grid1((size_t)h->L * kGroup, kBlock), dim3(kBlock), 0,
                    h->cam, h->L, h->lm_ptr.p, h->e_kf.p, h->e_uv.p, h->e_info.p, B.pa, h->fixed.p, B.la, h->Hpl.p,
@@ -4397,12 +4551,12 @@
             const bool lin = step && h->run_spec;
             FinArgs fin{1, (int)ug.x, h->P, h->O, h->root, step ? 1 : 0, 1, note ? 1 : 0, h->fixed.p, h->xp.p, h->bp.p, B.pa,
                         B.pb, h->o_i.p, h->o_j.p, h->o_meas.p, h->o_info.p, scal, h->d_mail, seq, h->ctl.p,
-                        (const volatile int*)h->d_stop, h->fin_counter.p, lin ? 1 : 0};
+                        (const volatile int*)h->d_stop, h->fin_counter.p, lin ? 1 : 0, lin ? h->run_repair : 0};
             if (lin)
-                SE2_LAUNCH(h->prof, st, "k_update_lin", k_update<true>, dim3(ug.x + 1), dim3(kBlock), 0, h->cam, h->L, 0.0, h->lm_ptr.p,
+                SE2_LAUNCH(h->prof, st, "k_update_lin", k_update<true>, dim3(ug.x + 1 + h->run_repair), dim3(kBlock), 0, h->cam, h->L, 0.0, h->lm_ptr.p,
                            h->e_kf.p, h->e_uv.p, h->e_info.p, B.pa, h->fixed.p, B.la, (const double*)h->xp.p,
                            h->z.p, (const double*)h->Hpl.p, h->bl.p, B.lb, h->part.p, B.c, B.pb, fin, (const double*)h->Dinv.p,
-                           SpecArgs{{rec_own(h), rec_twin(h)}, h->Hpp_e.p, h->bp_e.p});
+                           SpecArgs{{rec_own(h), rec_twin(h)}, h->Hpp_e.p, h->bp_e.p, rec_park(h, false), rec_park(h, true)});
             else
                 SE2_LAUNCH(h->prof, st, "k_update", k_update<false>, dim3(ug.x + 1), dim3(kBlock), 0, h->cam, h->L, 0.0, h->lm_ptr.p,
                            h->e_kf.p, h->e_uv.p, h->e_info.p, B.pa, h->fixed.p, B.la, step ? h->xp.p : (const double*)nullptr,
@@ -4437,7 +4591,7 @@
             SE2_CHECK(ba_reduce(h, 0.0, 0, true));
         }
     } else {
-        if (know_retry != 1) SE2_CHECK(ba_linearize(h, 0.0, true));
+        if (know_retry != 1 && !h->run_repair) SE2_CHECK(ba_linearize(h, 0.0, true));
         SE2_CHECK(ba_reduce(h, 0.0, !lm ? 0 : know_retry == 0 ? 0 : know_retry == 1 ? 3 : (h->model ? 2 : 0), true));
     }
     SE2_CHECK(ba_allreduce_system(h));
@@ -4726,6 +4880,7 @@
 
 void se2gpu_ba_destroy(se2gpu_ba* h) {
     if (!h) return;
+    ba_repair_release(h);
     if (h->join_event) { (void)hipEventSynchronize(h->join_event); h->join_event = nullptr; h->join_stream = nullptr; }
     if (ba_pool_enabled()) {
         (void)hipStreamSynchronize(h->stream);
@@ -5393,6 +5548,14 @@
     if (runs) *runs = c.lin_runs;
     if (skips) *skips = c.lin_skips;
     if (twin_bytes) *twin_bytes = (long long)(h->rec_twin.cap * sizeof(double));
+    return SE2GPU_OK;
+}
+
+int se2gpu_ba_debug_repair_workgroups(const se2gpu_ba* h, int* last_run, int* process_waiters, int* lin_launches) {
+    SE2_REQUIRE(h && h->initialized, SE2GPU_ERR_STATE, "debug_repair_workgroups before initialize");
+    if (last_run) *last_run = h->last_repair;
+    if (lin_launches) *lin_launches = h->run_lin_launches;
+    if (process_waiters) *process_waiters = g_repair_waiters.load(std::memory_order_relaxed);
     return SE2GPU_OK;
 }
 
@@ -5448,6 +5611,8 @@
     h->run_enqueued = 0;
     h->run_sync = sync;
     h->run_spec = false;
+    h->run_repair = h->last_repair = h->run_lin_launches = 0;
+    ba_repair_release(h);
     h->run_active = true;
     *h->h_stop = (stop_flag && *stop_flag) ? 1 : 0;
     return SE2GPU_OK;
@@ -5462,6 +5627,7 @@
     SE2_CHECK(ba_run_prologue(h, h->stream, nullptr, iters, mode, sync, stop_flag));
     h->run_spec = ba_env_speculate() && h->model == 0 && !h->allreduce && !h->comm && h->L > 0 && iters > 1;
     if (h->run_spec) SE2_CHECK(ba_reserve_twin(h));
+    if (h->run_spec && !h->run_sync) h->run_repair = h->last_repair = ba_repair_acquire(h);
     const int n0 = h->run_sync ? 1 : std::max(iters, 1);
     auto enqueue_all = [&]() -> int {
         hipLaunchKernelGGL(k_ctl_init, dim3(1), dim3(64), 0, h->stream, h->ctl.p, iters, mode);
@@ -5474,7 +5640,7 @@
     se2gpu_ba::GraphSlot* slot = nullptr;
     if (graphable) {
         for (auto& g : h->graphs)
-            if (g.iters == iters && g.mode == mode) slot = &g;
+            if (g.iters == iters && g.mode == mode && g.repair == h->run_repair) slot = &g;
         if (!slot) {
             slot = &h->graphs[0];
             for (auto& g : h->graphs)
@@ -5483,10 +5649,12 @@
             *slot = se2gpu_ba::GraphSlot{};
             slot->iters = iters;
             slot->mode = mode;
+            slot->repair = h->run_repair;
             slot->stamp = ++h->graph_clock;
             SE2_CHECK(enqueue_all());
         } else if (slot->exec) {
             slot->stamp = ++h->graph_clock;
+            h->run_lin_launches = slot->lin_launches;
             SE2_HIP(hipGraphLaunch(slot->exec, h->stream));
         } else {
             slot->stamp = ++h->graph_clock;
@@ -5496,6 +5664,7 @@
             const hipError_t ce = hipStreamEndCapture(h->stream, &g);
             SE2_CHECK(rc);
             SE2_HIP(ce);
+            slot->lin_launches = h->run_lin_launches;
             const hipError_t ie = hipGraphInstantiate(&slot->exec, g, nullptr, nullptr, 0);
             (void)hipGraphDestroy(g);
             SE2_HIP(ie);
@@ -5519,6 +5688,7 @@
     std::atomic_thread_fence(std::memory_order_acquire);
     BaCtl c;
     std::memcpy(&c, (const void*)(h->h_mail + 8), sizeof(BaCtl));
+    SE2_REQUIRE(c.error != 2, SE2GPU_ERR_HIP, "k_update: a repair workgroup never saw the finisher's verdict (2 s)");
     if (c.error && !h->chol_steps) {
         std::fprintf(stderr, "se2gpu_ba: k_chol_tiles timed out; continuing with k_chol_step\n");
         h->chol_steps = h->chol_fallback = true;
@@ -5552,6 +5722,7 @@
 
 int ba_run_finish(se2gpu_ba* h, se2gpu_ba_stats* stats) {
     h->own_pending = false;
+    ba_repair_release(h);
     BaCtl c;
     std::memcpy(&c, (const void*)(h->h_mail + 8), sizeof(BaCtl));
     h->run_active = false;
@@ -5582,6 +5753,7 @@
             if (hs[i]->run_active) {
                 (void)hipStreamSynchronize(hs[i]->stream);
                 hs[i]->run_active = false;
+                ba_repair_release(hs[i]);
             }
     }
 };
diff --git a/se2lam_amd/csrc/ba_device.h b/se2lam_amd/csrc/ba_device.h
--- a/se2lam_amd/csrc/ba_device.h
+++ b/se2lam_amd/csrc/ba_device.h
@@ -32,7 +32,7 @@
     int rec_sel, rec_valid, lin_runs, lin_skips;
     double seq;
     unsigned epoch;
-    unsigned pad2;
+    unsigned verdict;
 };
 
 __host__ __device__ inline double normalize_theta(double theta) {
diff --git a/se2lam_amd/optimizer.py b/se2lam_amd/optimizer.py
--- a/se2lam_amd/optimizer.py
+++ b/se2lam_amd/optimizer.py
@@ -109,6 +109,11 @@
         runs, skips, twin = C.c_int(0), C.c_int(0), C.c_longlong(0)
         capi.check(capi.lib().se2gpu_ba_debug_linearize_counts(self._h, C.byref(runs), C.byref(skips), C.byref(twin)))
         return int(runs.value), int(skips.value), int(twin.value)
+
+    def repair_workgroups(self):
+        last, waiters, lin = C.c_int(0), C.c_int(0), C.c_int(0)
+        capi.check(capi.lib().se2gpu_ba_debug_repair_workgroups(self._h, C.byref(last), C.byref(waiters), C.byref(lin)))
+        return int(last.value), int(waiters.value), int(lin.value)
 
     def activeRobustChi2(self) -> float:
         v = capi.lib().se2gpu_ba_chi2(self._h)
```

Result: no change. 6894 iters/s (-0.5%).
